# yabebalFantaye/MCEvidence

Hardware: AMD Instinct MI355X
Metric: knn_queries_per_sec (higher is better)
Workload: dtype f16 filter + f64 refine (exact f64 results)

## Files before the change

### mcevidence_amd/csrc/capi_common.hpp

```cpp
#pragma once
namespace {

thread_local char g_err[512] = "";
thread_local char g_last_kernel[256] = "";
thread_local int g_prof_on = 0;
thread_local std::vector<std::pair<hipEvent_t, hipEvent_t>> g_ev_pool;
thread_local size_t g_ev_used = 0;
thread_local size_t g_ev_calls = 0;
thread_local bool g_in_tail = false;
thread_local int g_split_depth = 0;
thread_local double g_last_prune_geom[3] = {0, 0, 0};
thread_local double g_last_flops_main = 0.0, g_last_flops_all = 0.0;
thread_local std::vector<std::pair<hipEvent_t, hipEvent_t>> g_evs_pool;
thread_local size_t g_evs_used = 0;

int fail(int code, const char* fmt, ...)
{
    va_list ap;
    va_start(ap, fmt);
    vsnprintf(g_err, sizeof(g_err), fmt, ap);
    va_end(ap);
    return code;
}

#define MCE_HIP(call)                                                                              \
    do {                                                                                           \
        hipError_t e_ = (call);                                                                    \
        if (e_ != hipSuccess)                                                                      \
            return fail(MCE_ERR_HIP, "%s failed: %s (%s:%d)", #call, hipGetErrorString(e_), __FILE__, __LINE__); \
    } while (0)

std::atomic<int> g_mode{0};
std::atomic<int> g_prune_mode{0};
struct Tuning {
    bool sym_kernel_f16 = false, tail_split = true, prune_prof = false, wide = true;
    int spin_limit = 1 << 21, sym_bucket = 0, sym_panel = 0, sym_seed_rows = 0, sym_seed_share = 2, sym_seed_mode = -1;
    int f16_seed_rows = -1, f16_seed_share = -1, f16_seed_tg = -1, rsplit = 0, panel_debug = 0, sym_chains = 0;
    size_t feed_wave_bytes = 0;
};
Tuning read_tuning()
{
    Tuning t;
    auto num = [](const char* name, int dflt) { const char* e = getenv(name); return e ? atoi(e) : dflt; };
    const char* e = getenv("MCE_SYM_KERNEL");
    t.sym_kernel_f16 = e && strcmp(e, "f16") == 0;
    t.spin_limit = num("MCE_SYM_SPIN_LIMIT", 1 << 21);
    t.sym_bucket = num("MCE_SYM_BUCKET", 0);
    t.sym_panel = num("MCE_SYM_PANEL", 0);
    t.sym_chains = num("MCE_SYM_CHAINS", 0);
    t.sym_seed_rows = num("MCE_SYM_SEED_ROWS", 0);
    t.sym_seed_share = num("MCE_SYM_SEED_SHARE", 2);
    t.sym_seed_mode = num("MCE_SYM_SEED_MODE", -1);
    t.f16_seed_rows = num("MCE_F16_SEED_ROWS", -1);
    t.f16_seed_share = num("MCE_F16_SEED_SHARE", -1);
    t.f16_seed_tg = num("MCE_F16_SEED_TG", -1);
    t.rsplit = num("MCE_RSPLIT", 0);
    t.tail_split = num("MCE_TAIL_SPLIT", 1) != 0;
    t.wide = num("MCE_WIDE", 1) != 0;
    t.panel_debug = num("MCE_PANEL_DEBUG", 0);
    t.prune_prof = getenv("MCE_PRUNE_PROF") != nullptr;
    if ((e = getenv("MCE_FEED_WAVE_BYTES"))) t.feed_wave_bytes = (size_t)std::strtoull(e, nullptr, 10);
    return t;
}
std::atomic<int> g_sym_mode{-1};
int sym_mode()
{
    int m = g_sym_mode.load();
    if (m < 0) {
        const char* e = getenv("MCE_SYM");
        m = e ? atoi(e) : 0;
        if (m < 0 || m > 2) m = 0;
        g_sym_mode.store(m);
    }
    return m;
}
const char* env_prune_heavy() { return getenv("MCE_PRUNE_HEAVY"); }
const char* env_prune_lists() { return getenv("MCE_PRUNE_LISTS"); }
const char* env_prune_times() { return getenv("MCE_PRUNE_TIMES"); }
bool env_long_on() { static const bool v = [] { const char* e = getenv("MCE_LONG"); return !(e && e[0] == '0'); }(); return v; }
bool env_deep_on() { static const bool v = [] { const char* e = getenv("MCE_DEEP"); return !(e && e[0] == '0'); }(); return v; }
int env_feed_eig() { static const int v = [] { const char* e = getenv("MCE_FEED_EIG"); return e && !strcmp(e, "hip") ? 2 : 1; }(); return v; }
bool env_feed_upload_async() { static const bool v = [] { const char* e = getenv("MCE_FEED_UPLOAD"); return e && !strcmp(e, "async"); }(); return v; }
int env_pairs_once_split() { static const int v = [] { const char* e = getenv("MCE_PAIRS_ONCE_SPLIT"); const int n = e ? atoi(e) : 0; return (n >= 1 && n <= 8) ? n : 0; }(); return v; }
int env_pairs_once_panel() { static const int v = [] { const char* e = getenv("MCE_PAIRS_ONCE_PANEL"); const int n = e ? atoi(e) : 0; return n >= 1 ? n : 0; }(); return v; }
struct CallOptions { int search = -1, prune = -1, sym = -1, same_set = -1, verify = -1, eig = 0; };
thread_local CallOptions t_opt;
thread_local std::vector<CallOptions> t_opt_stack;
int eff_search_mode() { return t_opt.search >= 0 ? t_opt.search : g_mode.load(); }
int eff_prune_mode() { return t_opt.prune >= 0 ? t_opt.prune : g_prune_mode.load(); }
int eff_sym_mode() { return t_opt.sym >= 0 ? t_opt.sym : sym_mode(); }
constexpr int kVerifyDefaultRows = 256;
constexpr int64_t kVerifyAlwaysFrom = 65536;
constexpr int kVerifySmallEvery = 8;
int default_verify_rows()
{
    static const int v = [] {
        const char* e = getenv("MCE_VERIFY");
        if (!e || !*e) return kVerifyDefaultRows;
        const long n = strtol(e, nullptr, 10);
        return (int)std::max<long>(0, std::min<long>(n, 1 << 20));
    }();
    return v;
}
bool verify_env_set() { static const bool s = [] { const char* e = getenv("MCE_VERIFY"); return e && *e; }(); return s; }
std::atomic<int> g_last_verify_rows{0};
thread_local unsigned t_small_search_count = 0;
int eff_verify(bool filter_path, int64_t nq)
{
    if (t_opt.verify >= 0) return t_opt.verify;
    if (!filter_path) return 0;
    if (nq < kVerifyAlwaysFrom && !verify_env_set() && (t_small_search_count++ % kVerifySmallEvery) != 0) return 0;
    return default_verify_rows();
}
constexpr int kSymAutoMinBlocks[5] = {0, 768, 257, 193, 193};
constexpr int kSymMaxChains = 8;
constexpr int kSymSeedMode[5] = {0, 0, 1, 1, 1};
constexpr int kSymPartitionMaxParts = 4;
thread_local int g_same_set_hint = -1;
thread_local size_t t_plan_cap = 0;
struct PlanCap {
    size_t prev;
    explicit PlanCap(size_t cap) : prev(t_plan_cap) { t_plan_cap = cap; }
    ~PlanCap() { t_plan_cap = prev; }
};
thread_local bool t_no_heavy = false;
struct NoHeavy {
    bool prev;
    NoHeavy() : prev(t_no_heavy) { t_no_heavy = true; }
    ~NoHeavy() { t_no_heavy = prev; }
};
struct SameSetHint {
    int prev;
    explicit SameSetHint(bool same) : prev(g_same_set_hint) { g_same_set_hint = same ? 1 : 0; }
    ~SameSetHint() { g_same_set_hint = prev; }
};
constexpr int kSymPanelChunks[5] = {0, 96, 256, 256, 256};
int sym_bucket_per_row(int K)
{
    const int b = read_tuning().sym_bucket;
    return b > 0 ? b : 6 * K + 24;
}
constexpr int64_t kPruneAutoMinQueries = 32768;
constexpr int64_t kPruneAutoMinRows[16] = {0, 100000, 100000, 100000, 100000, 125000, 150000, 250000, 500000, 0, 0, 0, 0, 0, 0, 0};

constexpr size_t kPoolMaxBytes = (size_t)64 << 20;
constexpr int kPoolSlots = 16;
struct PoolSlot { void* p = nullptr; size_t cap = 0; int dev = -1; bool busy = false; };
struct Pool {
    PoolSlot slot[kPoolSlots];
    PoolSlot& operator[](int i) { return slot[i]; }
    void release_idle()
    {
        for (int i = 0; i < kPoolSlots; ++i)
            if (slot[i].p && !slot[i].busy) {
                int cur = 0;
                (void)hipGetDevice(&cur);
                if (slot[i].dev != cur) (void)hipSetDevice(slot[i].dev);
                (void)hipFree(slot[i].p);
                if (slot[i].dev != cur) (void)hipSetDevice(cur);
                slot[i] = PoolSlot();
            }
    }
    ~Pool() { release_idle(); }
};
thread_local Pool g_pool;

struct PinnedArena {
    void* p = nullptr;
    size_t cap = 0;
    void release()
    {
        if (p) (void)hipHostFree(p);
        p = nullptr;
        cap = 0;
    }
    hipError_t reserve(size_t n)
    {
        if (n <= cap) return hipSuccess;
        release();
        const size_t c = std::max<size_t>(n + n / 2, (size_t)64 << 10);
        hipError_t e = hipHostMalloc(&p, c, hipHostMallocPortable);
        if (e != hipSuccess) { p = nullptr; return e; }
        cap = c;
        return hipSuccess;
    }
    ~PinnedArena() { release(); }
};
thread_local PinnedArena g_pinned;

thread_local const double* g_last_params = nullptr;

struct DevBuf {
    void* p = nullptr;
    int slot = -1;
    ~DevBuf()
    {
        if (p && g_last_params >= static_cast<const double*>(p) &&
            reinterpret_cast<const char*>(g_last_params) < static_cast<const char*>(p) + bytes)
            g_last_params = nullptr;
        if (slot >= 0) g_pool[slot].busy = false;
        else if (p) (void)hipFree(p);
    }
    size_t bytes = 0;
    hipError_t alloc(size_t n)
    {
        if (n == 0) n = 1;
        bytes = n;
        if (n <= kPoolMaxBytes) {
            int dev = 0;
            (void)hipGetDevice(&dev);
            int pick = -1;
            for (int i = 0; i < kPoolSlots; ++i)
                if (!g_pool[i].busy && g_pool[i].p && g_pool[i].dev == dev && g_pool[i].cap >= n &&
                    (pick < 0 || g_pool[i].cap < g_pool[pick].cap)) pick = i;
            if (pick < 0)
                for (int i = 0; i < kPoolSlots; ++i)
                    if (!g_pool[i].busy) {
                        if (g_pool[i].p) { (void)hipFree(g_pool[i].p); g_pool[i].p = nullptr; g_pool[i].cap = 0; }
                        const size_t cap = n + n / 4;
                        hipError_t e = hipMalloc(&g_pool[i].p, cap);
                        if (e != hipSuccess) { g_pool[i].p = nullptr; return e; }
                        g_pool[i].cap = cap;
                        g_pool[i].dev = dev;
                        pick = i;
                        break;
                    }
            if (pick >= 0) {
                g_pool[pick].busy = true;
                slot = pick;
                p = g_pool[pick].p;
                return hipSuccess;
            }
        }
        return hipMalloc(&p, n);
    }
    template <class T> T* as() { return static_cast<T*>(p); }
};

}
```

### mcevidence_amd/csrc/capi_plan.hpp

```cpp
#pragma once
namespace {

using mce::kMaxDevices;
constexpr int kAssumedCUs = 256;

size_t align_up(size_t x, size_t a) { return (x + a - 1) / a * a; }

constexpr bool kPruneHeavyDefault = false;
constexpr int kPruneHeavyMinBlocks = 64, kPruneHeavyCount = 700, kPruneHeavyMaxShare = 16, kPruneHeavyMinCount = 32, kPruneHeavyMaxRounds = 60;
constexpr double kPruneHeavyFullRounds = 10.0;
constexpr int kPruneHeavySplit = 4, kPruneHeavyMaxSplit = 8;
constexpr int kPruneWaveQueries = mce::kHQT * 32;
constexpr int kWideMinBlocks = 480;
bool prune_heavy_enabled()
{
    if (t_no_heavy) return false;
    const char* e = env_prune_heavy();
    return kPruneHeavyDefault || (e && *e && strcmp(e, "0") != 0);
}
static_assert(mce::kPruneWavesPerBlock == mce::kHWaves, "prune.hip orders kHWaves waves per query block");

constexpr int kRefineMargin = 2;
struct Plan {
    const mce::KnnVariant* v = nullptr;
    const mce::KnnF16Variant* vh = nullptr;
    const mce::KnnDeepVariant* vd = nullptr;
    bool filter() const { return vh != nullptr || vd != nullptr; }
    const mce::KnnLongVariant* vl = nullptr;
    size_t off_xf = 0, off_xn = 0;
    bool generic = false;
    int KST = 0;
    size_t off_yh = 0, off_xh = 0, off_qinfo = 0, off_params = 0;
    int KS = 0, KCAP = 0, QT = 0, CT = 0;
    int64_t nchunk = 0;
    int64_t nrow_pad = 0;
    int nqblk = 0;
    int64_t nq_pad = 0;
    int rsplit = 1;
    int L = 4;
    size_t off_yf = 0, off_pd = 0, off_pi = 0, off_center = 0, off_msum = 0, total = 0;
    double cost = 0.0;
    int ksel = 0;
    bool twopass = false;
    bool wide_ok = false;
    bool prune = false;
    bool kd_ready = false;
    int part = 0, nparts = 1;
    int sym_qb_lo = 0, sym_qb_hi = 0;
    bool apo = false;
    int apo_phase = 0;
    int apo_nsplit = 1;
    int apo_panel = 0;
    int64_t pl_nr = 0;
    mce::PruneLayout pl;
    size_t off_prune = 0;
    size_t off_heavy = 0;
    int heavy_max = 0;
    bool sym = false;
    bool sym_active = false;
    mce::SymLayout sl;
    size_t off_sym = 0;
    int sym_nsplit = 1;
    int sym_panel = 0;
};

const mce::KnnVariant* variant_for(int KS, int kcap_idx)
{
    switch (kcap_idx) {
        case 0: return &mce::g_knn_kcap4[mce::mfma_variant_index(KS)];
        case 1: return &mce::g_knn_kcap8[mce::mfma_variant_index(KS)];
        case 2: return &mce::g_knn_kcap12[mce::mfma_variant_index(KS)];
        case 3: return &mce::g_knn_kcap16[mce::mfma_variant_index(KS)];
        case 4: return &mce::g_knn_kcap24[mce::mfma_variant_index(KS)];
        default: return &mce::g_knn_kcap32[mce::mfma_variant_index(KS)];
    }
}

int sweep_seed_cfg(int64_t cps, int CT, int kneed)
{
    const Tuning t = read_tuning();
    if (t.f16_seed_rows >= 0 || t.f16_seed_share >= 0 || t.f16_seed_tg >= 0)
        return mce::f16_seed_cfg(cps, CT, kneed, t.f16_seed_rows >= 0 ? t.f16_seed_rows : MCE_H_SEED_ROWS, t.f16_seed_share >= 0 ? t.f16_seed_share : MCE_H_SEED_SHARE,
                                 t.f16_seed_tg >= 0 ? t.f16_seed_tg : MCE_H_SEED_TG);
    for (int share = MCE_H_SEED_SHARE; share >= 2; share /= 2)
        for (int tg = MCE_H_SEED_TG; tg >= 2; tg /= 2)
            if (const int cfg = mce::f16_seed_cfg(cps, CT, kneed, MCE_H_SEED_ROWS, share, tg)) return cfg;
    return 0;
}

template <class V> const V* by_kcap(int ki, const V* t4, const V* t8, const V* t12, const V* t16) { return ki == 0 ? t4 : ki == 1 ? t8 : ki == 2 ? t12 : t16; }

double split_cost(const Plan& p, bool filt, int64_t nr, int32_t K, int r)
{
    const double n_r = (double)nr / r;
    const double lnf = 1.0 + std::log(std::max(1.0, n_r / K));
    const double block = filt ? 64.0 * p.QT * p.KST * (n_r / 32.0) + 300.0 * 32.0 * p.QT * K * lnf
                              : 256.0 * p.KS * (n_r / 16.0) + 1000.0 * 32.0 * K * lnf;
    const double rounds = std::ceil((double)p.nqblk * r / kAssumedCUs);
    return rounds * block;
}

int make_plan(int64_t nq, int64_t nr, int32_t d, int32_t K, int32_t self_mode, Plan& p)
{
    if (nq < 0 || nr < 1 || d < 1 || K < 1) return fail(MCE_ERR_INVALID, "invalid sizes nq=%lld nr=%lld d=%d K=%d", (long long)nq, (long long)nr, d, K);
    if (self_mode < 0 || self_mode > 2) return fail(MCE_ERR_INVALID, "invalid self_mode %d", self_mode);
    if (d > mce::kGenMaxDim) return fail(MCE_ERR_DIM_RANGE, "d=%d exceeds the supported maximum %d", d, mce::kGenMaxDim);
    if (K > mce::kGenMaxK) return fail(MCE_ERR_K_RANGE, "K=%d exceeds the supported maximum %d", K, mce::kGenMaxK);
    const int64_t usable = (self_mode == MCE_SELF_EXCLUDE) ? nr - 1 : nr;
    if (K > usable)
        return fail(MCE_ERR_K_RANGE, "Expected n_neighbors <= n_samples_fit, but n_neighbors = %d, n_samples_fit = %lld", K, (long long)usable);
    if (nr >= (int64_t)1 << 31) return fail(MCE_ERR_INVALID, "nr=%lld exceeds 2^31-1 reference rows", (long long)nr);

    const bool wide_f64 = d > MCE_MAX_DIM && d <= mce::kWideMaxDim && K <= MCE_MAX_K;
    if (env_long_on() && d >= mce::kLongMinDim && d <= mce::kLongMaxDim && K <= MCE_MAX_K) {
        p.ksel = std::min<int>(K + kRefineMargin, MCE_MAX_K);
        p.vl = &mce::g_knn_long[p.ksel <= 8 ? 0 : (p.ksel <= 16 ? 1 : 2)];
        p.v = nullptr;
        p.vh = nullptr;
        p.KCAP = p.vl->kcap;
        p.CT = p.vl->ct;
        p.QT = mce::kLongQT;
        p.KS = mce::long_ksp(d);
        p.nqblk = (int)std::max<int64_t>(1, (nq + mce::kLongQPB - 1) / mce::kLongQPB);
        p.nq_pad = (int64_t)p.nqblk * mce::kLongQPB;
        const int64_t rows_per_chunk = (int64_t)p.CT * 16;
        p.nchunk = (nr + rows_per_chunk - 1) / rows_per_chunk;
        p.nrow_pad = p.nchunk * rows_per_chunk;
        int best_r = 1;
        double best_c = 1e300;
        const int rmax = (int)std::min<int64_t>(mce::kMaxLists, p.nchunk);
        for (int r = 1; r <= rmax; ++r) {
            const double c = std::ceil((double)p.nqblk * r / kAssumedCUs) * (std::ceil((double)p.nchunk / r) + 16.0);
            if (c < best_c * 0.98) { best_c = c; best_r = r; }
        }
        p.rsplit = best_r;
        p.L = p.rsplit;
        p.cost = best_c;
        p.pl_nr = nr;
        size_t off = 0;
        p.off_pd = off;
        off = align_up(off + (size_t)p.L * p.KCAP * (size_t)p.nq_pad * sizeof(double), 256);
        p.off_pi = off;
        off = align_up(off + (size_t)p.L * p.KCAP * (size_t)p.nq_pad * sizeof(int), 256);
        p.off_center = off;
        off = align_up(off + (size_t)(d + 4) * sizeof(double), 256);
        p.off_msum = off;
        off = align_up(off + (size_t)mce::kLongMeanBlocks * (size_t)d * sizeof(double), 256);
        p.off_yf = off;
        off = align_up(off + (size_t)p.nrow_pad * (size_t)p.KS * 4 * sizeof(double), 256);
        p.off_xf = off;
        off = align_up(off + (size_t)p.nq_pad * (size_t)p.KS * 4 * sizeof(double), 256);
        p.off_xn = off;
        off = align_up(off + (size_t)p.nq_pad * sizeof(double), 256);
        p.total = off + 256;
        return MCE_OK;
    }
    if ((d > MCE_MAX_DIM && !wide_f64) || K > MCE_MAX_K) {
        p.generic = true;
        p.v = nullptr;
        p.vh = nullptr;
        p.KCAP = K;
        p.rsplit = 1;
        p.L = 1;
        p.nqblk = (int)std::max<int64_t>(1, (nq + mce::kGenThreads - 1) / mce::kGenThreads);
        p.nq_pad = (int64_t)p.nqblk * mce::kGenThreads;
        size_t off = 0;
        p.off_pd = off;
        off = align_up(off + (size_t)K * (size_t)p.nq_pad * sizeof(double), 256);
        p.off_pi = off;
        off = align_up(off + (size_t)K * (size_t)p.nq_pad * sizeof(int), 256);
        p.off_center = off;
        off = align_up(off + (size_t)nq * K * sizeof(double), 256);
        p.off_msum = off;
        p.total = off + 256;
        return MCE_OK;
    }
    p.KS = mce::mfma_ks_for(d);
    int ki = 0;
    while (ki < mce::kNumKcap - 1 && mce::kKcapList[ki] < K) ++ki;
    p.KCAP = mce::kKcapList[ki];
    const bool f16 = !wide_f64 && (eff_search_mode() != 1) && mce::f16_supported(d, K);
    const bool deep = wide_f64 && (eff_search_mode() != 1) && mce::deep_supported(d, K) && env_deep_on();
    const bool filt = f16 || deep;
    p.vd = nullptr;
    int qpb, rows_per_tile;
    if (filt) {
        if (K > 16) {
            p.twopass = true;
            ki = 3;
            p.KCAP = 16;
        }
        if (deep) {
            p.KST = mce::deep_ksteps(d);
            p.vd = &by_kcap(ki, mce::g_knn_deep_kcap4, mce::g_knn_deep_kcap8, mce::g_knn_deep_kcap12, mce::g_knn_deep_kcap16)[p.KST == 5 ? 0 : (p.KST == 6 ? 1 : 2)];
            p.vh = nullptr;
            p.QT = mce::kHQT;
            p.CT = p.vd->ct;
        } else {
            p.KST = mce::f16_ksteps(d);
            p.vh = &by_kcap(ki, mce::g_knn_f16_kcap4, mce::g_knn_f16_kcap8, mce::g_knn_f16_kcap12, mce::g_knn_f16_kcap16)[p.KST - 1];
            p.QT = p.vh->qt;
            p.CT = p.vh->ct;
        }
        p.v = nullptr;
        qpb = mce::f16_qpb(p.KCAP);
        rows_per_tile = 32;
    } else {
        p.ksel = std::min<int>(K + kRefineMargin, MCE_MAX_K);
        p.pl_nr = nr;
        ki = 0;
        while (ki < mce::kNumKcap - 1 && mce::kKcapList[ki] < p.ksel) ++ki;
        p.KCAP = mce::kKcapList[ki];
        p.v = variant_for(p.KS, ki);
        p.vh = nullptr;
        p.QT = p.v->qt;
        p.CT = p.v->ct;
        qpb = mce::queries_per_block(p.QT);
        rows_per_tile = 16;
    }
    p.nqblk = (int)std::max<int64_t>(1, (nq + qpb - 1) / qpb);
    p.wide_ok = f16 && !p.twopass && p.KST == 1 && p.vh->launch_wide && p.nqblk >= kWideMinBlocks && nr <= ((int64_t)1 << 25) && read_tuning().wide;
    if (p.wide_ok && (p.nqblk & 1)) p.nqblk += 1;
    p.nq_pad = (int64_t)p.nqblk * qpb;
    const int64_t rows_per_chunk = (int64_t)p.CT * rows_per_tile;
    p.nchunk = (nr + rows_per_chunk - 1) / rows_per_chunk;
    p.nrow_pad = p.nchunk * rows_per_chunk;

    if (f16 && !p.twopass && p.KST == 1 && d <= mce::kPruneMaxDim && p.vh->launch_prune && nq > 0 &&
        p.nrow_pad <= ((int64_t)1 << mce::kHRelBits) && (int64_t)p.nqblk * p.nchunk <= mce::kPruneMaxPairs) {
        const int pm = eff_prune_mode();
        p.prune = pm == 2 || (pm == 0 && kPruneAutoMinRows[d] > 0 && nr >= kPruneAutoMinRows[d] && nq >= kPruneAutoMinQueries &&
                                           nq >= nr / 8);
    }
    if (p.prune) {
        p.CT = mce::kHPruneChunkTiles;
        p.nchunk = (nr + p.CT * 32 - 1) / (p.CT * 32);
        p.nrow_pad = p.nchunk * p.CT * 32;
        if (p.nrow_pad > ((int64_t)1 << mce::kHRelBits)) p.prune = false;
        if (!p.prune) {
            p.CT = p.vh->ct;
            p.nchunk = (nr + rows_per_chunk - 1) / rows_per_chunk;
            p.nrow_pad = p.nchunk * rows_per_chunk;
        }
    }
    int best_r = 1;
    double best_c = 1e300;
    const int rmax = (int)std::min<int64_t>(p.twopass ? mce::kMaxLists / 2 : mce::kMaxLists, p.nchunk);
    const int rmin = f16 ? (int)((nr + ((int64_t)1 << mce::kHRelBits) - 1) >> mce::kHRelBits) : 1;
    if (deep && p.nrow_pad > ((int64_t)1 << mce::kHRelBits))
        return fail(MCE_ERR_INVALID, "reference set too large for the fp16-filter path at d = %d (nr=%lld): use search mode 1", d, (long long)nr);
    if (rmin > rmax) return fail(MCE_ERR_INVALID, "reference set too large for the fp16-filter path (nr=%lld)", (long long)nr);
    for (int r = std::max(1, rmin); r <= rmax; ++r) {
        const double c = split_cost(p, filt, nr, K, r);
        if (c < best_c * 0.98) { best_c = c; best_r = r; }
    }
    if (f16 && !p.twopass && p.nqblk <= kAssumedCUs) {
        const int kneed = K + 1;
        for (int r = std::min(rmax, kAssumedCUs / p.nqblk); r >= std::max(1, rmin); --r)
            if (sweep_seed_cfg(p.nchunk / r, p.CT, kneed)) { best_r = r; break; }
    }
    if (deep && p.nqblk <= kAssumedCUs) {
        for (int r = std::min(rmax, kAssumedCUs / p.nqblk); r >= 1; --r)
            if ((p.nchunk / r) * p.CT >= 4 * (K + 1)) { best_r = r; break; }
    }
    if (const int r = read_tuning().rsplit) {
        if (r >= std::max(1, rmin) && r <= rmax) best_r = r;
    }
    if (p.prune) best_r = 1;
    p.rsplit = best_r;
    p.cost = split_cost(p, filt, nr, K, best_r);
    auto layout = [&]() {
    p.L = p.twopass ? 2 * p.rsplit : p.rsplit;

    size_t off = 0;
    p.off_yf = off;
    if (filt) {
        p.off_yh = off;
        off = align_up(off + (size_t)p.nrow_pad * (size_t)(16 * p.KST) * 2, 256);
        p.off_xh = off;
        off = align_up(off + (size_t)p.nq_pad * (size_t)(16 * p.KST) * 2, 256);
        p.off_qinfo = off;
        off = align_up(off + (size_t)p.nq_pad * 2 * sizeof(double), 256);
        p.off_params = off;
        off = align_up(off + (size_t)mce::HP_COUNT * sizeof(double), 256);
    } else {
        off = align_up(off + (size_t)p.nrow_pad * (size_t)(4 * p.KS) * sizeof(double), 256);
    }
    if (f16 && (!p.twopass || p.vh->launch_panel_lower) && !p.prune && nq == nr && p.vh->launch_sym && p.nqblk >= 2 && p.nrow_pad <= ((int64_t)1 << mce::kHSymRowBits)) {
        const int sm = eff_sym_mode();
        p.sym = sm == 2 || (sm == 0 && p.nqblk >= kSymAutoMinBlocks[p.KST] * ((p.KST == 1 && p.KCAP == 16) ? 2 : 1));
        if (g_same_set_hint == 0 || (g_same_set_hint < 0 && t_opt.same_set == 0)) p.sym = false;
    }
    p.sym_nsplit = 1;
    p.sym_panel = 0;
    if (p.sym && !p.twopass) {
        const Tuning tun = read_tuning();
        int S = 1;
        if (tun.sym_chains >= 1) S = std::min(tun.sym_chains, kSymMaxChains);
        p.sym_nsplit = S;
        if (S > 1) p.sym_panel = (int)std::max<int64_t>(8, std::min<int64_t>(kSymPanelChunks[p.KST], p.nchunk / (2 * S)));
    }
    const int l_alloc = std::max(p.L, p.sym_nsplit);
    p.off_pd = off;
    off = align_up(off + (size_t)l_alloc * p.KCAP * (size_t)p.nq_pad * sizeof(double), 256);
    p.off_pi = off;
    off = align_up(off + (size_t)l_alloc * p.KCAP * (size_t)p.nq_pad * sizeof(int), 256);
    p.off_center = off;
    off = align_up(off + (size_t)3 * mce::kMaxDimPad * sizeof(double), 256);
    p.off_msum = off;
    off = align_up(off + (size_t)mce::kMeanBlocks * mce::kStatStride * sizeof(double), 256);
    if (p.prune) {
        mce::prune_layout(nq, p.nq_pad, p.nqblk, nr, p.nrow_pad, p.nchunk, d, p.pl);
        p.pl_nr = nr;
        p.off_prune = off;
        off = align_up(off + p.pl.total, 256);
        if (nq == nr && p.nqblk >= kPruneHeavyMinBlocks && prune_heavy_enabled()) {
            p.heavy_max = std::max(p.nqblk * mce::kHWaves / kPruneHeavyMaxShare, kPruneHeavyMinCount);
            p.off_heavy = off;
            off = align_up(off + (size_t)p.heavy_max * kPruneWaveQueries * (kPruneHeavyMaxSplit - 1) * p.KCAP * (sizeof(double) + sizeof(int)), 256);
        }
    }
    if (p.sym) {
        mce::sym_layout(nr, p.nq_pad, p.nqblk, d, p.KCAP, mce::f16_qpb(p.KCAP), sym_bucket_per_row(std::min<int>(K, p.KCAP)), p.sl);
        p.off_sym = off;
        off = align_up(off + p.sl.total, 256);
    }
    p.total = off;
    };
    layout();
    while (t_plan_cap && p.total > t_plan_cap && p.rsplit > std::max(1, rmin)) {
        p.rsplit -= 1;
        layout();
    }
    return MCE_OK;
}

size_t dotp_ws_bytes(int64_t nq, int32_t kmax)
{
    const int64_t nb = (nq + mce::kRedThreads - 1) / mce::kRedThreads;
    return align_up((size_t)std::max<int64_t>(nb, 1) * (size_t)kmax * sizeof(double), 256);
}

int plan_for_workspace(int64_t nq, int64_t nr, int32_t d, int32_t K, int32_t self_mode, size_t ws_bytes, size_t extra, bool same_set_fallback,
                       Plan& p, std::optional<NoHeavy>& nh)
{
    int rc = make_plan(nq, nr, d, K, self_mode, p);
    if (rc != MCE_OK) return rc;
    if (same_set_fallback && ws_bytes < p.total + extra && p.sym) {
        g_same_set_hint = 0;
        rc = make_plan(nq, nr, d, K, self_mode, p);
        if (rc != MCE_OK) return rc;
    }
    if (ws_bytes < p.total + extra && p.heavy_max > 0) {
        nh.emplace();
        rc = make_plan(nq, nr, d, K, self_mode, p);
        if (rc != MCE_OK) return rc;
    }
    if (ws_bytes < p.total + extra) return fail(MCE_ERR_WORKSPACE, "workspace too small: %zu < %zu", ws_bytes, p.total + extra);
    return MCE_OK;
}

}
```

### mcevidence_amd/csrc/capi_search.hpp

```cpp
#pragma once
namespace {

double ln_unit_ball(int d) { return 0.5 * d * std::log(M_PI) - std::lgamma(1.0 + 0.5 * d); }

hipError_t launch_sym_merge(int KCAP, double* pd, int* pi, int64_t nq_pad, const mce::SymParams& sym, int qb_lo, int qb_hi, hipStream_t st, int stride = 1)
{
    const int nb = qb_hi > qb_lo ? (qb_hi - qb_lo + stride - 1) / stride : 0;
    if (nb <= 0) return hipSuccess;
    const dim3 g((unsigned)nb), b(mce::kSymMergeThreads);
    static_assert(mce::kSymMergeThreads == mce::f16_qpb(4), "one merge block per query block");
    switch (KCAP) {
        case 4: hipLaunchKernelGGL(mce::sym_merge_kernel<4>, g, b, 0, st, pd, pi, nq_pad, sym.bucket_cnt, sym.bucket_flag, sym.bucket, sym.cap, qb_lo, stride); break;
        case 8: hipLaunchKernelGGL(mce::sym_merge_kernel<8>, g, b, 0, st, pd, pi, nq_pad, sym.bucket_cnt, sym.bucket_flag, sym.bucket, sym.cap, qb_lo, stride); break;
        case 12: hipLaunchKernelGGL(mce::sym_merge_kernel<12>, g, b, 0, st, pd, pi, nq_pad, sym.bucket_cnt, sym.bucket_flag, sym.bucket, sym.cap, qb_lo, stride); break;
        default: hipLaunchKernelGGL(mce::sym_merge_kernel<16>, g, b, 0, st, pd, pi, nq_pad, sym.bucket_cnt, sym.bucket_flag, sym.bucket, sym.cap, qb_lo, stride); break;
    }
    return hipGetLastError();
}

struct KernelBracket {
    bool on = false; hipStream_t st = nullptr;
    hipError_t begin() const
    {
        if (!on) return hipSuccess;
        if (g_ev_used == g_ev_pool.size()) {
            hipEvent_t e0, e1;
            if (const hipError_t e = hipEventCreate(&e0)) return e;
            if (const hipError_t e = hipEventCreate(&e1)) return e;
            g_ev_pool.emplace_back(e0, e1);
        }
        return hipEventRecord(g_ev_pool[g_ev_used].first, st);
    }
    hipError_t end() const
    {
        if (!on) return hipSuccess;
        if (const hipError_t e = hipEventRecord(g_ev_pool[g_ev_used].second, st)) return e;
        ++g_ev_used;
        if (!g_in_tail) ++g_ev_calls;
        return hipSuccess;
    }
};
struct SearchBracket {
    hipStream_t st; bool on;
    SearchBracket(hipStream_t s, bool o) : st(s), on(o)
    {
        if (!on) return;
        if (g_evs_used == g_evs_pool.size()) {
            hipEvent_t e0, e1;
            if (hipEventCreate(&e0) != hipSuccess || hipEventCreate(&e1) != hipSuccess) { on = false; return; }
            g_evs_pool.emplace_back(e0, e1);
        }
        (void)hipEventRecord(g_evs_pool[g_evs_used].first, st);
    }
    ~SearchBracket() { if (on) { (void)hipEventRecord(g_evs_pool[g_evs_used].second, st); ++g_evs_used; } }
};

size_t list_set(const Plan& p, int set) { return (size_t)set * p.KCAP * (size_t)p.nq_pad; }

mce::KnnF16Args f16_args(const Plan& p, char* ws, const double* X, int64_t nq, const double* Y, int64_t nr, int32_t d, int32_t K, int self_exclude,
                         int64_t self_offset)
{
    mce::KnnF16Args a;
    a.Yh = ws + p.off_yh; a.nchunk_total = p.nchunk; a.rsplit = p.rsplit; a.Xh = ws + p.off_xh;
    a.qinfo = reinterpret_cast<const double*>(ws + p.off_qinfo); a.params = reinterpret_cast<const double*>(ws + p.off_params);
    a.X = X; a.Y = Y; a.nq = nq; a.nr = nr; a.D = d; a.nq_pad = p.nq_pad; a.nqblk = p.nqblk;
    a.self_exclude = self_exclude; a.self_offset = self_offset; a.ksel = K;
    a.part_d = reinterpret_cast<double*>(ws + p.off_pd); a.part_i = reinterpret_cast<int*>(ws + p.off_pi);
    return a;
}
mce::KnnF16Args sym_args(const Plan& p, char* ws, int64_t n, int32_t d, int32_t K, int self_exclude)
{
    char* const sw = ws + p.off_sym;
    const double* rows = reinterpret_cast<const double*>(sw + p.sl.Ys);
    mce::KnnF16Args a = f16_args(p, ws, rows, n, rows, n, d, K, self_exclude, 0);
    a.rsplit = 1;
    a.rperm = reinterpret_cast<const int*>(sw + p.sl.perm);
    a.sym.thr = reinterpret_cast<unsigned long long*>(sw + p.sl.thr);
    a.sym.rrow = reinterpret_cast<unsigned*>(sw + p.sl.rrow);
    a.sym.rtile = reinterpret_cast<float*>(sw + p.sl.rtile);
    a.sym.slots = reinterpret_cast<unsigned long long*>(sw + p.sl.slots);
    a.sym.bucket_cnt = reinterpret_cast<int*>(sw + p.sl.bucket_cnt);
    a.sym.bucket_flag = reinterpret_cast<int*>(sw + p.sl.bucket_flag);
    a.sym.bucket = reinterpret_cast<mce::SymEntry*>(sw + p.sl.bucket);
    a.sym.cap = p.sl.cap;
    a.sym.done = reinterpret_cast<int*>(sw + p.sl.done);
    const Tuning tun = read_tuning();
    a.sym.panel = tun.sym_panel > 0 ? tun.sym_panel : kSymPanelChunks[p.KST];
    return a;
}

struct F16Search {
    const double* sX = nullptr;
    const double* sY = nullptr;
    mce::PruneOut po;
    bool use_sym = false;
};

struct Search {
    Plan& p;
    const double* dX; int64_t nq; const double* dY; int64_t nr; int32_t d, K;
    int32_t self_mode; int64_t self_offset; char* ws; hipStream_t st;
    int phase;
    double* pd; int* pi;
    double* center; double* msum;
    int self_exclude;
    KernelBracket kb;
    int generic(), long_rows(), deep(), fp64();
    int f16_prepare(F16Search& f), pruned(const F16Search& f), symmetric(), f16_sweep(const F16Search& f);
};

int Search::generic()
{
    const size_t lds = mce::generic_lds_bytes();
    hipLaunchKernelGGL(mce::knn_generic_kernel, dim3((unsigned)p.nqblk), dim3(mce::kGenThreads), 0, st, dX, nq, dY, nr, (int)d,
                       (int)K, p.nq_pad, self_exclude, self_offset, pd, pi);
    MCE_HIP(hipGetLastError());
    snprintf(g_last_kernel, sizeof(g_last_kernel), "knn_generic_kernel grid=%d block=%d lds=%zu", p.nqblk, mce::kGenThreads, lds);
    return MCE_OK;
}

int Search::long_rows()
{
    const int threads = 256;
    double* yf = reinterpret_cast<double*>(ws + p.off_yf);
    double* xf = reinterpret_cast<double*>(ws + p.off_xf);
    double* xn = reinterpret_cast<double*>(ws + p.off_xn);
    hipLaunchKernelGGL(mce::pack_refs_kernel, dim3((unsigned)((p.nrow_pad + threads - 1) / threads)), dim3(threads), 0, st, dY, nr, (int)d, p.KS, p.nrow_pad, center, yf);
    MCE_HIP(hipGetLastError());
    const int64_t qe = p.nq_pad * (int64_t)p.KS;
    hipLaunchKernelGGL(mce::long_pack_queries_kernel, dim3((unsigned)((qe + 255) / 256)), dim3(256), 0, st, dX, nq, (int)d, p.KS, p.nq_pad, center, xf);
    MCE_HIP(hipGetLastError());
    hipLaunchKernelGGL(mce::long_query_norms_kernel, dim3((unsigned)((p.nq_pad + 255) / 256)), dim3(256), 0, st, dX, nq, (int)d, p.nq_pad, center, xn);
    MCE_HIP(hipGetLastError());
    mce::LongArgs a;
    a.Yf = yf; a.Xf = xf; a.xn = xn;
    a.nchunk_total = p.nchunk; a.rsplit = p.rsplit; a.KSP = p.KS; a.KSB = mce::long_ksb(d);
    a.nq = nq; a.nq_pad = p.nq_pad; a.nqblk = p.nqblk;
    a.self_exclude = self_exclude; a.self_offset = self_offset; a.ksel = p.ksel > K ? p.ksel : K;
    a.part_d = pd; a.part_i = pi;
    MCE_HIP(kb.begin());
    MCE_HIP(p.vl->launch(a, st));
    MCE_HIP(kb.end());
    snprintf(g_last_kernel, sizeof(g_last_kernel), "%s grid=%d block=%d lds=%zu qt=%d ct=%d rsplit=%d ksp=%d", p.vl->name, p.nqblk * p.rsplit, mce::kThreads,
             p.vl->lds_bytes, p.QT, p.CT, p.rsplit, p.KS);
    g_last_flops_main = g_last_flops_all = (double)p.nq_pad * (double)p.nrow_pad * 2.0 * 4.0 * p.KS;
    return MCE_OK;
}

int Search::deep()
{
    _Float16* yh = reinterpret_cast<_Float16*>(ws + p.off_yh);
    _Float16* xh = reinterpret_cast<_Float16*>(ws + p.off_xh);
    double* qinfo = reinterpret_cast<double*>(ws + p.off_qinfo);
    double* params = reinterpret_cast<double*>(ws + p.off_params);
    MCE_HIP(mce::zero_async(params, mce::HP_COUNT * sizeof(double), st));
    const bool separate_queries = !(dX >= dY && dX + (size_t)nq * d <= dY + (size_t)nr * d);
    hipLaunchKernelGGL(mce::f16_radius_rows_kernel, dim3((unsigned)std::min<int64_t>((nr + 255) / 256, 2048)), dim3(256), 0, st, dY, nr, (int)d, center, params);
    MCE_HIP(hipGetLastError());
    if (separate_queries && nq > 0) {
        hipLaunchKernelGGL(mce::f16_radius_rows_kernel, dim3((unsigned)std::min<int64_t>((nq + 255) / 256, 2048)), dim3(256), 0, st, dX, nq, (int)d, center, params);
        MCE_HIP(hipGetLastError());
    }
    hipLaunchKernelGGL(mce::f16_scale_from_radius_kernel, dim3(1), dim3(1), 0, st, params);
    MCE_HIP(hipGetLastError());
    const int64_t rows_per_block = 4 * (64 / (2 * p.KST));
    const int64_t pack_blocks = std::min<int64_t>((p.nrow_pad + rows_per_block - 1) / rows_per_block, 2048);
    hipLaunchKernelGGL(mce::f16_pack_refs_kernel, dim3((unsigned)pack_blocks), dim3(256), 0, st, dY, nr, (int)d, p.KST, p.nrow_pad, center, params, yh);
    MCE_HIP(hipGetLastError());
    hipLaunchKernelGGL(mce::f16_pack_queries_kernel, dim3((unsigned)((p.nq_pad + rows_per_block - 1) / rows_per_block)), dim3(256), 0, st,
                       dX, nq, p.nq_pad, (int)d, p.KST, center, params, xh, qinfo);
    MCE_HIP(hipGetLastError());
    mce::DeepArgs a;
    a.Yh = yh; a.Xh = xh; a.qinfo = qinfo; a.params = params; a.X = dX; a.Y = dY; a.part_d = pd; a.part_i = pi;
    a.nq = nq; a.nr = nr; a.nq_pad = p.nq_pad; a.self_offset = self_offset; a.nchunk_total = p.nchunk;
    a.D = d; a.ksel = K; a.self_exclude = self_exclude; a.nqblk = p.nqblk; a.rsplit = p.rsplit;
    const Tuning tun = read_tuning();
    a.debug = tun.panel_debug;
    const int64_t tiles_split = (p.nchunk / p.rsplit) * p.CT;
    const int64_t want = (tun.f16_seed_rows >= 0 ? tun.f16_seed_rows : MCE_H_SEED_ROWS) / 32;
    auto tg_for = [&](int G) {
        int64_t tg = std::min<int64_t>(want, tiles_split / 4) / G;
        if (tg < 1) tg = std::min<int64_t>(want, tiles_split / 2) / G;
        return (int)std::max<int64_t>(tg, 0);
    };
    a.seed_tg = tg_for(K + a.self_exclude);
    MCE_HIP(kb.begin());
    double seed_rows = (double)a.seed_tg * (K + a.self_exclude) * 32.0 * p.rsplit;
    if (p.twopass) {
        const int tg2 = a.seed_tg;
        a.ksel = 16;
        a.seed_groups = 16 + a.self_exclude;
        a.seed_tg = tg_for(a.seed_groups);
        const int tg1 = a.seed_tg;
        MCE_HIP(p.vd->launch(a, st));
        a.lo_d = pd; a.lo_i = pi;
        a.part_d = pd + list_set(p, p.rsplit); a.part_i = pi + list_set(p, p.rsplit);
        a.ksel = K - 16;
        a.seed_groups = K + a.self_exclude;
        a.seed_tg = tg2;
        MCE_HIP(p.vd->launch_lower(a, st));
        seed_rows = ((double)tg1 * (16 + a.self_exclude) + (double)tg2 * (K + a.self_exclude)) * 32.0 * p.rsplit;
    } else {
        MCE_HIP(p.vd->launch(a, st));
    }
    MCE_HIP(kb.end());
    g_last_flops_main = g_last_flops_all = (double)p.nq_pad * ((p.twopass ? 2.0 : 1.0) * (double)p.nrow_pad + seed_rows) * 2.0 * 16.0 * p.KST;
    snprintf(g_last_kernel, sizeof(g_last_kernel), "%s grid=%d block=%d lds=%zu qt=%d ct=%d rsplit=%d%s seed=%dx%d", p.vd->name, p.nqblk * p.rsplit, mce::kHThreads,
             p.vd->lds_bytes, p.QT, p.CT, p.rsplit, p.twopass ? " two passes" : "", K + a.self_exclude, a.seed_tg);
    return MCE_OK;
}

int Search::f16_prepare(F16Search& f)
{
    _Float16* yh = reinterpret_cast<_Float16*>(ws + p.off_yh);
    _Float16* xh = reinterpret_cast<_Float16*>(ws + p.off_xh);
    double* qinfo = reinterpret_cast<double*>(ws + p.off_qinfo);
    double* params = reinterpret_cast<double*>(ws + p.off_params);
    double* box_y = center + mce::kMaxDimPad;
    double* box_x = center + 2 * mce::kMaxDimPad;
    if (phase != 2) MCE_HIP(mce::zero_async(params, mce::HP_COUNT * sizeof(double), st));
    bool separate_queries = !(dX >= dY && dX + (size_t)nq * d <= dY + (size_t)nr * d);
    f.sX = dX; f.sY = dY;
    f.use_sym = p.sym && dX == dY && nq == nr && self_offset == 0 && g_split_depth == 0;
    if (f.use_sym) {
        if (phase != 2) MCE_HIP(mce::sym_prepare(dY, nr, (int)d, center, p.nq_pad, ws + p.off_sym, p.sl, st));
        f.sX = f.sY = reinterpret_cast<const double*>(ws + p.off_sym + p.sl.Ys);
        separate_queries = false;
    }
    if (p.prune) {
        const bool same_set = (dX == dY && nq == nr);
        MCE_HIP(mce::prune_prepare(dX, nq, dY, nr, (int)d, same_set, mce::f16_qpb(p.KCAP), p.CT * 32, p.nq_pad, p.nqblk, p.nrow_pad,
                                   p.nchunk, ws + p.off_prune, p.pl, st, f.po, p.kd_ready && same_set));
        f.sX = f.po.Xs; f.sY = f.po.Ys;
        separate_queries = separate_queries && !same_set;
    }
    if (separate_queries) {
        hipLaunchKernelGGL(mce::col_stats_partial_kernel, dim3(mce::kMeanBlocks), dim3(mce::kMeanThreads), 0, st, dX, nq, (int)d, msum);
        MCE_HIP(hipGetLastError());
        hipLaunchKernelGGL(mce::f16_box_about_kernel, dim3(1), dim3(64), 0, st, msum, (int)d, center, box_x);
        MCE_HIP(hipGetLastError());
    }
    if (phase == 2) return MCE_OK;
    hipLaunchKernelGGL(mce::f16_scale_kernel, dim3(1), dim3(64), 0, st, box_y, separate_queries ? box_x : (const double*)nullptr, params);
    MCE_HIP(hipGetLastError());
    const int64_t rows_per_block = 4 * (64 / (2 * p.KST));
    const int64_t pack_blocks = std::min<int64_t>((p.nrow_pad + rows_per_block - 1) / rows_per_block, 2048);
    const bool one_pass = f.sX == f.sY && nq == nr && p.nq_pad <= p.nrow_pad;
    hipLaunchKernelGGL(mce::f16_pack_refs_kernel, dim3((unsigned)pack_blocks), dim3(256), 0, st,
                       f.sY, nr, (int)d, p.KST, p.nrow_pad, center, params, yh, one_pass ? xh : (_Float16*)nullptr, one_pass ? qinfo : (double*)nullptr,
                       one_pass ? p.nq_pad : (int64_t)0);
    MCE_HIP(hipGetLastError());
    if (!one_pass) {
        hipLaunchKernelGGL(mce::f16_pack_queries_kernel, dim3((unsigned)((p.nq_pad + rows_per_block - 1) / rows_per_block)), dim3(256), 0, st,
                           f.sX, nq, p.nq_pad, (int)d, p.KST, center, params, xh, qinfo);
        MCE_HIP(hipGetLastError());
    }
    return MCE_OK;
}

int Search::pruned(const F16Search& f)
{
    const mce::PruneOut& po = f.po;
    mce::KnnF16Args a = f16_args(p, ws, f.sX, nq, f.sY, nr, d, K, self_exclude, self_offset);
    a.clist = po.clist; a.cdist = po.cdist; a.list_len = (int)p.nchunk; a.rperm = po.rperm; a.qperm = po.qperm;
    a.tbox_r = po.tbox_r; a.tbox_q = po.tbox_q; a.cbox_r = po.cbox_r; a.border = po.border;
    const int nw_total = p.nqblk * mce::kHWaves;
    if (p.nparts > 1) { a.qblk0 = p.part; a.qblk_stride = p.nparts; a.nqblk_run = (nw_total - p.part + p.nparts - 1) / p.nparts; }
    const int nblk_run = a.nqblk_run ? a.nqblk_run : nw_total;
    int hv_n = 0, hv_S = 1;
    if (p.heavy_max > 0 && dX == dY && nq == nr) {
        const double rounds = (double)nblk_run / 2048.0;
        const char* hv_env = env_prune_heavy();
        if ((kPruneHeavyDefault || (hv_env && !strcmp(hv_env, "auto"))) && rounds < kPruneHeavyMaxRounds) {
            const double fr = std::min(1.0, kPruneHeavyFullRounds / std::max(rounds, 1.0));
            hv_n = std::min(std::max((int)(kPruneHeavyCount * fr), kPruneHeavyMinCount), std::min(p.heavy_max, nblk_run));
            hv_S = kPruneHeavySplit;
        }
        if (const char* e = hv_env) {
            int n_ = hv_n, s_ = kPruneHeavySplit;
            if (sscanf(e, "%d,%d", &n_, &s_) >= 1) { hv_n = std::min(std::max(n_, 0), std::min(p.heavy_max, nblk_run)); hv_S = std::min(std::max(s_, 1), kPruneHeavyMaxSplit); }
        }
        if (hv_n == 0 || hv_S == 1) { hv_n = 0; hv_S = 1; }
    }
    double* hv_d = reinterpret_cast<double*>(ws + p.off_heavy);
    int* hv_i = reinterpret_cast<int*>(hv_d + (size_t)p.heavy_max * kPruneWaveQueries * (kPruneHeavyMaxSplit - 1) * p.KCAP);
    a.seed_cfg = hv_n | (hv_S << 24);
    a.lo_d = hv_n ? hv_d : nullptr; a.lo_i = hv_n ? hv_i : nullptr;
    const char* times_file = env_prune_times();
    const size_t n_wg = (size_t)(nblk_run + hv_n * (hv_S - 1));
    DevBuf wg_times;
    if (times_file && *times_file) { MCE_HIP(wg_times.alloc(n_wg * sizeof(float))); a.wg_us = wg_times.as<float>(); }
    MCE_HIP(kb.begin());
    const char* force_lists = env_prune_lists();
    mce::knn_f16_launch_fn short_fn = nullptr;
    int short_lc = 0;
    if (p.vh->launch_prune_short && K <= p.vh->prune_short_lc) { short_fn = p.vh->launch_prune_short; short_lc = p.vh->prune_short_lc; }
    else if (p.vh->launch_prune_short2 && K <= p.vh->prune_short_lc2) { short_fn = p.vh->launch_prune_short2; short_lc = p.vh->prune_short_lc2; }
    const bool short_lists = short_fn && !(force_lists && !strcmp(force_lists, "long"));
    MCE_HIP(short_lists ? short_fn(a, st) : p.vh->launch_prune(a, st));
    MCE_HIP(kb.end());
    if (a.wg_us) {
        std::vector<float> us(n_wg);
        MCE_HIP(hipStreamSynchronize(st));
        MCE_HIP(hipMemcpy(us.data(), a.wg_us, n_wg * sizeof(float), hipMemcpyDeviceToHost));
        if (FILE* fh = fopen(times_file, "wb")) {
            const int hdr[4] = {(int)n_wg, hv_n, hv_S, 1};
            fwrite(hdr, sizeof(int), 4, fh);
            fwrite(us.data(), sizeof(float), n_wg, fh);
            fclose(fh);
        }
    }
    if (hv_n) {
        const unsigned fb = (unsigned)(((int64_t)hv_n * kPruneWaveQueries + mce::kRedThreads - 1) / mce::kRedThreads);
        hipLaunchKernelGGL(mce::prune_heavy_fold_kernel, dim3(fb), dim3(mce::kRedThreads), 0, st, pd, pi, p.nq_pad, p.KCAP, hv_d, hv_i, hv_n, hv_S,
                           kPruneWaveQueries, po.border, a.qblk0, a.qblk_stride);
        MCE_HIP(hipGetLastError());
    }
    g_last_params = a.params;
    g_last_flops_main = g_last_flops_all = -1.0;
    g_last_prune_geom[0] = p.nqblk; g_last_prune_geom[1] = (double)p.nchunk; g_last_prune_geom[2] = p.CT;
    snprintf(g_last_kernel, sizeof(g_last_kernel), "%s pruned grid=%d block=64 lds=%zu qt=%d ct=%d chunks=%lld heavy=%dx%d lists=%d", p.vh->name,
             nblk_run + hv_n * (hv_S - 1), mce::f16_prune_lds_bytes(p.KST, d, short_lists ? short_lc : p.KCAP), p.QT, p.CT, (long long)p.nchunk, hv_n,
             hv_S, short_lists ? short_lc : p.KCAP);
    return MCE_OK;
}

int sym_units_and_flops(const Plan& p, const mce::PanelGeom& g, bool panel_kernel, int64_t nr, int panel)
{
    int units = mce::sym_unit_count(p.nqblk, mce::kHWaves * mce::kHQT, panel * p.CT, (int)((nr + 31) / 32) + (int)(((nr + 31) / 32) & 1));
    double tiles = 0.0;
    if (panel_kernel) {
        units = mce::panel_unit_count(g);
        for (int u = 0; g_prof_on && u < units; ++u) {
            int pp, aa, lo, hi;
            mce::panel_unit_decode(u, g, pp, aa);
            mce::panel_unit_tiles(pp, aa, g, lo, hi);
            tiles += hi - lo;
        }
    } else {
        const double tpb = mce::kHWaves * mce::kHQT, T = (double)((nr + 31) / 32);
        for (int b = 0; b < p.nqblk; ++b) tiles += std::min(tpb * (b + 1), T);
    }
    g_last_flops_main = tiles * 16.0 * 1024.0 * 32.0 * p.KST;
    return units;
}

int Search::symmetric()
{
    char* const sw = ws + p.off_sym;
    mce::KnnF16Args a = sym_args(p, ws, nr, d, K, self_exclude);
    const Tuning tun = read_tuning();
    const int seed_rows = tun.sym_seed_rows > 0 ? tun.sym_seed_rows : (p.KST == 1 ? 65536 : 32768) * (p.apo && p.nparts >= 4 ? 2 : 1);
    const int seed_share = tun.sym_seed_share;
    auto sym_seed_for = [&](int kk) {
        int cfg = mce::f16_seed_cfg(p.nchunk, p.CT, kk + a.self_exclude, seed_rows, seed_share, MCE_H_SEED_TG);
        for (int tg = MCE_H_SEED_TG / 2; cfg == 0 && tg >= 1; tg /= 2)
            cfg = mce::f16_seed_cfg(p.nchunk, p.CT, kk + a.self_exclude, seed_rows, seed_share, tg);
        if (cfg) cfg |= ((tun.sym_seed_mode >= 0 ? tun.sym_seed_mode : kSymSeedMode[p.KST]) & 3) << 28;
        return cfg;
    };
    const int qb_lo = p.nparts > 1 && !p.apo ? (int)((int64_t)p.nqblk * p.part / p.nparts) : 0;
    const int qb_hi = p.nparts > 1 && !p.apo ? (int)((int64_t)p.nqblk * (p.part + 1) / p.nparts) : p.nqblk;
    p.sym_qb_lo = qb_lo; p.sym_qb_hi = qb_hi;
    const bool panel_kernel = !tun.sym_kernel_f16 || p.nparts > 1 || p.twopass;
    mce::PanelGeom geom;
    geom.qb_lo = qb_lo; geom.qb_hi = qb_hi; geom.tpb = mce::kHWaves * mce::kHQT; geom.ct = p.CT; geom.tpp = a.sym.panel * p.CT; geom.sym_on = 1;
    geom.ntiles = (int)((nr + 31) / 32) + (int)(((nr + 31) / 32) & 1);
    const bool apo = p.apo && p.nparts > 1 && !p.twopass && panel_kernel;
    const bool chains1 = !apo && p.nparts == 1 && panel_kernel && !p.twopass && p.sym_nsplit > 1;
    if (apo) { geom.blk_first = p.part; geom.blk_stride = p.nparts; }
    if (apo || chains1) {
        const int pn = apo ? p.apo_panel : p.sym_panel;
        if (pn > 0 && (apo || tun.sym_panel <= 0)) { a.sym.panel = pn; geom.tpp = a.sym.panel * p.CT; }
        geom.nsplit = std::max(1, apo ? p.apo_nsplit : p.sym_nsplit);
        if (geom.nsplit > 1) {
            a.sym.done = reinterpret_cast<int*>(sw + p.sl.keys_b);
            MCE_HIP(mce::zero_async(a.sym.done, (size_t)p.nqblk * geom.nsplit * sizeof(int), st));
            if (!apo) {
                hipLaunchKernelGGL(mce::sym_chain_init_kernel, dim3((unsigned)p.nqblk), dim3(512), 0, st, pd, pi, p.nq_pad, p.KCAP, geom.nsplit, 0, 1);
                MCE_HIP(hipGetLastError());
            }
        }
    }
    const bool unit_table = apo || geom.nsplit > 1;
    const int npass = p.twopass ? 2 : 1;
    int seed_used = 0;
    for (int pass = 0; pass < npass; ++pass) {
        const bool lower = pass == 1;
        const int Kp = !p.twopass ? K : (lower ? K - 16 : 16);
        double* const pdp = pd + (lower ? list_set(p, 1) : 0);
        int* const pip = pi + (lower ? list_set(p, 1) : 0);
        if (lower) {
            MCE_HIP(mce::zero_async(a.sym.bucket_cnt, (size_t)3 * p.nqblk * sizeof(int), st));
            a.sym.slot_stride = p.KCAP;
        }
        a.ksel = lower ? K : Kp;
        a.seed_cfg = sym_seed_for(a.ksel);
        a.part_d = pdp; a.part_i = pip;
        a.qblk0 = qb_lo;
        a.nqblk_run = qb_hi - qb_lo;
        if (apo) {
            a.qblk0 = p.part; a.qblk_stride = p.nparts; a.nqblk_run = mce::apo_rank_count(p.nqblk, p.part, p.nparts);
        }
        if (a.nqblk_run > 0 && phase != 2) MCE_HIP((lower ? p.vh->launch_sym_pre32 : p.vh->launch_sym_pre)(a, st));
        a.qblk0 = 0; a.qblk_stride = 1; a.nqblk_run = 0;
        if (phase == 1) return MCE_OK;
        if (pass == 0) seed_used = a.seed_cfg;
        a.seed_cfg = 0;
        a.ksel = Kp;
        a.lo_d = lower ? pd : nullptr; a.lo_i = lower ? pi : nullptr;
        if (pass == 0) MCE_HIP(kb.begin());
        if (panel_kernel) {
            mce::PanelArgs pa;
            pa.Yh = static_cast<const _Float16*>(a.Yh); pa.Xh = static_cast<const _Float16*>(a.Xh); pa.qinfo = a.qinfo; pa.params = a.params;
            pa.X = a.X; pa.Y = a.Y; pa.rperm = a.rperm;
            pa.part_d = pdp; pa.part_i = pip; pa.nq = nq; pa.nr = nr; pa.nq_pad = p.nq_pad; pa.self_offset = 0;
            pa.D = d; pa.ksel = Kp; pa.self_exclude = a.self_exclude; pa.spin_limit = tun.spin_limit;
            pa.sym = a.sym; pa.debug = tun.panel_debug; pa.geom = geom; pa.lo_d = a.lo_d; pa.lo_i = a.lo_i;
            if (unit_table) {
                const int nun = mce::panel_unit_count(geom);
                if ((size_t)nun * sizeof(mce::PanelUnit) > (size_t)p.nq_pad * sizeof(int)) return fail(MCE_ERR_INVALID, "symmetric sweep: %d units do not fit the table", nun);
                mce::PanelUnit* tab = reinterpret_cast<mce::PanelUnit*>(sw + p.sl.vals_a);
                if (nun > 0) {
                    hipLaunchKernelGGL(mce::panel_unit_table_kernel, dim3((unsigned)((nun + 255) / 256)), dim3(256), 0, st, geom, nun, tab);
                    MCE_HIP(hipGetLastError());
                }
                pa.units = tab;
            }
            MCE_HIP((lower ? p.vh->launch_panel_lower : p.vh->launch_panel)(pa, st));
        } else {
            MCE_HIP(p.vh->launch_sym(a, st));
        }
        if (pass == 0) MCE_HIP(kb.end());
        if (apo) break;
        MCE_HIP((lower ? p.vh->launch_sym_repair_lower : p.vh->launch_sym_repair)(a, st));
        if (geom.nsplit > 1) {
            hipLaunchKernelGGL(mce::sym_chain_clear_kernel, dim3((unsigned)p.nqblk), dim3(512), 0, st, a.sym.bucket_flag, pdp, pip, p.nq_pad, p.KCAP, geom.nsplit, 0, 1);
            MCE_HIP(hipGetLastError());
        }
        MCE_HIP(launch_sym_merge(p.KCAP, pdp, pip, p.nq_pad, a.sym, qb_lo, qb_hi, st));
    }
    p.sym_active = true;
    p.L = geom.nsplit > 1 ? geom.nsplit : npass;
    const int sym_units = sym_units_and_flops(p, geom, panel_kernel, nr, a.sym.panel);
    g_last_flops_all = g_last_flops_main + (double)(seed_used & 0xffff) * p.CT * (double)(qb_hi - qb_lo) * 16.0 * 1024.0 * 32.0 * p.KST;
    snprintf(g_last_kernel, sizeof(g_last_kernel), "%s symmetric%s%s%s grid=%d block=%d lds=%zu qt=%d ct=%d panel=%d seed=%dx%d/%d bucket=%d", p.vh->name, panel_kernel ? " panel-kernel" : "",
             p.twopass ? " two passes" : "", geom.blk_stride > 1 ? " pairs-once" : (geom.nsplit > 1 ? " chains" : ""), sym_units,
             mce::kHThreads, panel_kernel ? p.vh->lds_bytes_panel : p.vh->lds_bytes_sym, p.QT, p.CT, a.sym.panel, seed_used & 0xffff, (seed_used >> 16) & 0xfff, (seed_used >> 28) & 3, p.sl.cap);
    return MCE_OK;
}

int Search::f16_sweep(const F16Search& f)
{
    mce::KnnF16Args a = f16_args(p, ws, f.sX, nq, f.sY, nr, d, K, self_exclude, self_offset);
    auto seed_cfg = [&](int ksel) { return sweep_seed_cfg(p.nchunk / p.rsplit, p.CT, ksel + a.self_exclude); };
    MCE_HIP(kb.begin());
    if (p.twopass) {
        a.ksel = 16;
        a.seed_cfg = seed_cfg(16);
        MCE_HIP(p.vh->launch(a, st));
        a.lo_d = pd; a.lo_i = pi;
        a.part_d = pd + list_set(p, p.rsplit); a.part_i = pi + list_set(p, p.rsplit);
        a.ksel = K - 16;
        a.seed_cfg = 0;
        MCE_HIP(p.vh->launch_lower(a, st));
    } else {
        a.seed_cfg = seed_cfg(K);
        if (p.wide_ok) MCE_HIP(p.vh->launch_wide(a, st));
        else MCE_HIP(p.vh->launch(a, st));
    }
    MCE_HIP(kb.end());
    const int seed_first = p.twopass ? seed_cfg(16) : a.seed_cfg;
    g_last_flops_main = (double)p.nqblk * ((double)p.nchunk + (double)(seed_first & 0xffff) * p.rsplit) * p.CT * 16.0 * 1024.0 * 32.0 * p.KST +
                        (p.twopass ? (double)p.nqblk * (double)p.nchunk * p.CT * 16.0 * 1024.0 * 32.0 * p.KST : 0.0);
    g_last_flops_all = g_last_flops_main;
    char seed_txt[48] = "";
    if (seed_first) snprintf(seed_txt, sizeof(seed_txt), " seed=%dx%d", seed_first & 0xffff, seed_first >> 16);
    const bool wide = p.wide_ok && !p.twopass;
    snprintf(g_last_kernel, sizeof(g_last_kernel), "%s grid=%d block=%d lds=%zu qt=%d ct=%d rsplit=%d%s%s%s", p.vh->name,
             (wide ? p.nqblk / 2 : p.nqblk) * p.rsplit, mce::kHThreads, wide ? p.vh->lds_bytes_wide : p.vh->lds_bytes, wide ? 2 * p.QT : p.QT, p.CT, p.rsplit,
             p.twopass ? " two passes" : "", seed_txt, wide ? " wide" : "");
    return MCE_OK;
}

int Search::fp64()
{
    const int threads = 256;
    double* yf = reinterpret_cast<double*>(ws + p.off_yf);
    hipLaunchKernelGGL(mce::pack_refs_kernel, dim3((unsigned)((p.nrow_pad + threads - 1) / threads)), dim3(threads), 0, st, dY, nr,
                       (int)d, p.KS, p.nrow_pad, center, yf);
    MCE_HIP(hipGetLastError());
    mce::KnnArgs a;
    a.Yf = yf; a.nchunk_total = p.nchunk; a.rsplit = p.rsplit; a.X = dX; a.center = center; a.nq = nq; a.D = d;
    a.nq_pad = p.nq_pad; a.nqblk = p.nqblk; a.self_exclude = self_exclude; a.self_offset = self_offset;
    a.ksel = p.ksel > K ? p.ksel : K;
    a.part_d = pd; a.part_i = pi;
    MCE_HIP(kb.begin());
    MCE_HIP(p.v->launch(a, st));
    MCE_HIP(kb.end());
    snprintf(g_last_kernel, sizeof(g_last_kernel), "%s grid=%d block=%d lds=%zu qt=%d ct=%d rsplit=%d", p.v->name,
             p.nqblk * p.rsplit, mce::kThreads, p.v->lds_bytes, p.QT, p.CT, p.rsplit);
    g_last_flops_main = g_last_flops_all = (double)p.nq_pad * (double)p.nrow_pad * 2.0 * 4.0 * p.KS;
    return MCE_OK;
}

int run_search(Plan& p, const double* dX, int64_t nq, const double* dY, int64_t nr, int32_t d, int32_t K,
               int32_t self_mode, int64_t self_offset, char* ws, hipStream_t st)
{
    p.sym_active = false;
    const int phase = p.apo ? p.apo_phase : 0;
    double* center = reinterpret_cast<double*>(ws + p.off_center);
    double* msum = reinterpret_cast<double*>(ws + p.off_msum);
    Search s{p, dX, nq, dY, nr, d, K, self_mode, self_offset, ws, st, phase, reinterpret_cast<double*>(ws + p.off_pd), reinterpret_cast<int*>(ws + p.off_pi),
             center, msum, (self_mode == MCE_SELF_EXCLUDE) ? 1 : 0, KernelBracket{}};
    if (p.generic) return s.generic();
    if (p.vl) {
        hipLaunchKernelGGL(mce::long_col_mean_partial_kernel, dim3(mce::kLongMeanBlocks), dim3(256), 0, st, dY, nr, (int)d, mce::kLongMeanBlocks, msum);
        MCE_HIP(hipGetLastError());
        hipLaunchKernelGGL(mce::long_col_mean_final_kernel, dim3((unsigned)((d + 255) / 256)), dim3(256), 0, st, msum, nr, (int)d, mce::kLongMeanBlocks, center);
        MCE_HIP(hipGetLastError());
    } else if (d > MCE_MAX_DIM) {
        static_assert(3 * mce::kMaxDimPad >= 128 && mce::kStatStride >= 128, "wide column means");
        hipLaunchKernelGGL(mce::col_mean_wide_partial_kernel, dim3(mce::kMeanBlocks), dim3(256), 0, st, dY, nr, (int)d, msum);
        MCE_HIP(hipGetLastError());
        hipLaunchKernelGGL(mce::col_mean_wide_final_kernel, dim3(1), dim3(128), 0, st, msum, nr, (int)d, center);
        MCE_HIP(hipGetLastError());
    } else if (phase != 2) {
        hipLaunchKernelGGL(mce::col_stats_partial_kernel, dim3(mce::kMeanBlocks), dim3(mce::kMeanThreads), 0, st, dY, nr, (int)d, msum);
        MCE_HIP(hipGetLastError());
        hipLaunchKernelGGL(mce::col_stats_final_kernel, dim3(1), dim3(64), 0, st, msum, nr, (int)d, center, center + mce::kMaxDimPad);
        MCE_HIP(hipGetLastError());
    }
    const bool prof = g_prof_on && g_ev_used < 1024;
    SearchBracket search_bracket(st, prof && g_evs_used < 1024);
    g_last_flops_main = g_last_flops_all = 0.0;
    s.kb = KernelBracket{prof, st};
    if (p.vl) return s.long_rows();
    if (p.vd) return s.deep();
    if (!p.vh) return s.fp64();
    F16Search f;
    const int rc = s.f16_prepare(f);
    if (rc != MCE_OK) return rc;
    if (p.prune) return s.pruned(f);
    return f.use_sym ? s.symmetric() : s.f16_sweep(f);
}

int launch_merge(const Plan& p, bool write_dist, bool fuse, const double* dX, const double* dY, int64_t nq, int32_t d, int K,
                 int self_mode, int64_t self_offset, double* d_dist, int64_t* d_idx, int k0, int kmax,
                 const double* d_w, const double* d_fs, double* partial, char* ws, hipStream_t st)
{
    const bool same_set = (dX == dY && nq == p.pl_nr);
    const bool wave_parts = p.prune && p.nparts > 1 && !p.sym_active;
    const int qpb = wave_parts ? kPruneWaveQueries : (p.filter() ? mce::f16_qpb(p.KCAP) : 1);
    const int nunits = wave_parts ? p.nqblk * mce::kHWaves : p.nqblk;
    int64_t ncol = nq;
    int64_t col0 = 0, col1 = INT64_MAX;
    const int* border = p.prune ? reinterpret_cast<const int*>(ws + p.off_prune + p.pl.border) : nullptr;
    if (p.sym_active && p.nparts > 1 && p.apo) {
        ncol = (int64_t)((nunits - p.part + p.nparts - 1) / p.nparts) * qpb;
        border = reinterpret_cast<const int*>(ws + p.off_sym + p.sl.done);
    } else if (p.sym_active && p.nparts > 1) {
        col0 = (int64_t)p.sym_qb_lo * qpb;
        col1 = std::min<int64_t>((int64_t)p.sym_qb_hi * qpb, nq);
        ncol = std::max<int64_t>(col1 - col0, 0);
    } else if (p.nparts > 1) ncol = (int64_t)((nunits - p.part + p.nparts - 1) / p.nparts) * qpb;
    const unsigned blocks = (unsigned)std::max<int64_t>((ncol + mce::kRedThreads - 1) / mce::kRedThreads, 1);
    const double* pd = reinterpret_cast<const double*>(ws + p.off_pd);
    const int* pi = reinterpret_cast<const int*>(ws + p.off_pi);
    const bool refine = !p.filter() && !p.generic;
    const double lnc = fuse ? ln_unit_ball(d) : 0.0;
    const int* qperm = nullptr;
    if (p.prune) qperm = reinterpret_cast<const int*>(ws + p.off_prune + (same_set ? p.pl.perm_r : p.pl.perm_q));
    if (p.sym_active) qperm = reinterpret_cast<const int*>(ws + p.off_sym + p.sl.perm);
#define MCE_MERGE(W, F, R)                                                                                          \
    hipLaunchKernelGGL((mce::merge_lists_kernel<W, F, R>), dim3(blocks), dim3(mce::kRedThreads), 0, st, pd, pi, p.L,  \
                       p.KCAP, nq, p.nq_pad, dX, dY, (int)d, K, (refine && p.ksel > K) ? p.ksel : K, self_mode, self_offset, d_dist, d_idx, K, k0, kmax, \
                       d_w, d_fs, lnc, partial, qperm, p.part, p.nparts, qpb, border, nunits, col0, col1, p.pl_nr, \
                       refine ? reinterpret_cast<const double*>(ws + p.off_center) : nullptr)
    if (write_dist && !fuse) { if (refine) MCE_MERGE(true, false, true); else MCE_MERGE(true, false, false); }
    else if (write_dist && fuse) { if (refine) MCE_MERGE(true, true, true); else MCE_MERGE(true, true, false); }
    else { if (refine) MCE_MERGE(false, true, true); else MCE_MERGE(false, true, false); }
#undef MCE_MERGE
    MCE_HIP(hipGetLastError());
    return MCE_OK;
}

int finish_dotp(const double* partial, int64_t ncols, int k0, int kmax, double* d_dotp, hipStream_t st)
{
    const unsigned blocks = (unsigned)std::max<int64_t>((ncols + mce::kRedThreads - 1) / mce::kRedThreads, 1);
    hipLaunchKernelGGL(mce::dotp_final_kernel, dim3((unsigned)kmax), dim3(mce::kRedThreads), 0, st, partial, (int64_t)blocks, k0, kmax, d_dotp);
    MCE_HIP(hipGetLastError());
    return MCE_OK;
}
int zero_dotp(double* d_dotp, int kmax, hipStream_t st) { MCE_HIP(mce::zero_async(d_dotp, (size_t)kmax * sizeof(double), st)); return MCE_OK; }

}
```

### mcevidence_amd/csrc/f16_filter.hpp

```cpp
#pragma once
#include <math.h>
#include <stdint.h>
#if defined(__HIPCC__)
#include <hip/hip_runtime.h>
#endif

#include "sym_types.hpp"

namespace mce {

#if defined(__HIPCC__)
#define MCE_HDI __host__ __device__ __forceinline__
#else
#define MCE_HDI inline
#endif

enum { HP_RMAX = 0, HP_SCALE = 1, HP_EY = 2, HP_YHATMAX = 3, HP_RHO = 4, HP_STAT_CHUNKS = 5, HP_STAT_TILES = 6, HP_COUNT = 16 };

constexpr int kHWaves = 8;
constexpr int kHThreads = kHWaves * 64;
constexpr int kHRelBits = 26;
constexpr int kHSymRowBits = kHRelBits - 1;

MCE_HDI float f16_round_up(double g)
{
#if defined(__HIP_DEVICE_COMPILE__)
    return __double2float_ru(g);
#else
    float f = (float)g;
    if ((double)f < g) f = nextafterf(f, __builtin_huge_valf());
    return f;
#endif
}
struct F16GateTerms { double a, c, eps; };
MCE_HDI double f16_gate_a(double ex, double ey, int KST) { return (ex + ey) * (1.0 + 1e-9) + 2.0 * sqrt(16.0 * KST) * 0x1p-14; }
MCE_HDI F16GateTerms f16_gate_terms(double ex, double xn, double ey, double ymax, double rho, int KST, bool live = true)
{
    const double r = sqrt(xn) + ymax;
    const double a = f16_gate_a(ex, ey, KST);
    const double eps = (32.0 * KST) * 0x1p-24 * r * r * (1.0 + 0x1p-9) + rho + 1e-30;
    return {a, live ? eps - xn : -__builtin_huge_val(), eps};
}
MCE_HDI double f16_reach2(double thr, double s2, double a)
{
    const double rr = sqrt(thr * s2) * (1.0 + 1e-12) + a;
    return rr * rr * (1.0 + 1e-12);
}
MCE_HDI float f16_gate_finite(double thr, double s2, double a, double c) { return f16_round_up(f16_reach2(thr, s2, a) + c); }
MCE_HDI float f16_gate(double thr, double s2, double a, double c)
{
    if (!(c > -__builtin_huge_val())) return -__builtin_huge_valf();
    if (!(thr < __builtin_huge_val())) return __builtin_huge_valf();
    return f16_gate_finite(thr, s2, a, c);
}
MCE_HDI double f16_row_const(double ymax) { return 0x1p-22 * (ymax * ymax + 1.0); }
MCE_HDI float f16_row_round(double g, double rowc) { return f16_round_up(g * (1.0 + 0x1p-22) + rowc + 1e-30); }
MCE_HDI float f16_row_gate(double thr, double s2, double a, double rowc)
{
    if (!(thr < __builtin_huge_val())) return __builtin_huge_valf();
    return f16_row_round(f16_reach2(thr, s2, a), rowc);
}
template <class P>
MCE_HDI float f16_row_gate_of(double thr, double ex, P params, int KST)
{
    if (!(thr < __builtin_huge_val())) return __builtin_huge_valf();
    const double s2 = params[HP_SCALE] * params[HP_SCALE];
    const double g = f16_reach2(thr, s2, f16_gate_a(ex, params[HP_EY], KST));
    return f16_row_round(g, f16_row_const(params[HP_YHATMAX]));
}
MCE_HDI double f16_seed_bound(double a_up, double xn, double eps, double a, double s2)
{
    const double dd = sqrt(fmax(a_up + xn + eps, 0.0)) * (1.0 + 1e-12) + a;
    return dd * dd * (1.0 + 1e-12) / s2 * (1.0 + 1e-12);
}

template <int N, class D, class I>
MCE_HD inline void list_insert(D&& own_d, I&& own_i, double d2, int j)
{
    const double INF = __builtin_huge_val();
    bool c_hi = (d2 < own_d[N - 1]) || (d2 == own_d[N - 1] && j < own_i[N - 1] && d2 < INF);
#pragma unroll
    for (int k = N - 1; k >= 1; --k) {
        const bool c_lo = (d2 < own_d[k - 1]) || (d2 == own_d[k - 1] && j < own_i[k - 1] && d2 < INF);
        own_d[k] = c_lo ? own_d[k - 1] : (c_hi ? d2 : own_d[k]);
        own_i[k] = c_lo ? own_i[k - 1] : (c_hi ? j : own_i[k]);
        c_hi = c_lo;
    }
    own_d[0] = c_hi ? d2 : own_d[0];
    own_i[0] = c_hi ? j : own_i[0];
}

#if defined(__HIPCC__)
typedef _Float16 v8h __attribute__((ext_vector_type(8)));
typedef float v16f __attribute__((ext_vector_type(16)));

__device__ __forceinline__ float min3f(float a, float b, float c)
{
    float r;
    asm("v_min3_f32 %0, %1, %2, %3" : "=v"(r) : "v"(a), "v"(b), "v"(c));
    return r;
}
__device__ __forceinline__ void f16_min16_halves(const v16f& c, float (&l1)[5], float& m0, float& m3)
{
    l1[0] = min3f(c[0], c[1], c[2]);
    l1[1] = min3f(c[3], c[4], c[5]);
    l1[2] = min3f(c[6], c[7], c[8]);
    l1[3] = min3f(c[9], c[10], c[11]);
    l1[4] = min3f(c[12], c[13], c[14]);
    m0 = min3f(l1[0], l1[1], l1[2]);
    m3 = min3f(l1[3], l1[4], c[15]);
}
__device__ __forceinline__ float f16_min16(const v16f& c, float (&l1)[5])
{
    float m0, m3;
    f16_min16_halves(c, l1, m0, m3);
    return min3f(m0, m3, m3);
}
__device__ __forceinline__ float f16_min16(const v16f& c, float (&l1)[5], float run)
{
    float m0, m3;
    f16_min16_halves(c, l1, m0, m3);
    return min3f(run, m0, m3);
}

template <int KCAP, class PS, class PT, class PR, class PF, class RG>
__device__ __forceinline__ bool sym_slot_insert(PS slots, PT thr, PR rrow, PF rtile, int ksel, int row, double d2, RG row_gate)
{
    const auto sl = slots + (int64_t)row * KCAP;
    for (;;) {
        double vmax = -1.0, v2 = -1.0;
        int imax = 0;
#pragma unroll
        for (int k = 0; k < KCAP; ++k) {
            if (k < ksel) {
                const double v = __longlong_as_double((long long)__hip_atomic_load(sl + k, __ATOMIC_RELAXED, __HIP_MEMORY_SCOPE_AGENT));
                if (v > vmax) { v2 = vmax; vmax = v; imax = k; }
                else if (v > v2) v2 = v;
            }
        }
        if (d2 > vmax) return false;
        if (d2 == vmax) return true;
        unsigned long long expect = (unsigned long long)__double_as_longlong(vmax);
        if (__hip_atomic_compare_exchange_strong(sl + imax, &expect, (unsigned long long)__double_as_longlong(d2), __ATOMIC_RELAXED,
                                                 __ATOMIC_RELAXED, __HIP_MEMORY_SCOPE_AGENT)) {
            const double nk = fmax(v2, d2);
            if (nk < __builtin_huge_val()) {
                const unsigned long long nb = (unsigned long long)__double_as_longlong(nk);
                const unsigned long long ob = __hip_atomic_fetch_min(thr + row, nb, __ATOMIC_RELAXED, __HIP_MEMORY_SCOPE_AGENT);
                if (nb < ob) {
                    const unsigned rb = __float_as_uint(row_gate(nk, row));
                    const unsigned orb = __hip_atomic_fetch_min(rrow + row, rb, __ATOMIC_RELAXED, __HIP_MEMORY_SCOPE_AGENT);
                    if (rb < orb) {
                        const auto rt = rrow + (int64_t)(row >> 5) * 32;
                        unsigned m = 0;
                        for (int k = 0; k < 32; ++k) {
                            const unsigned v = __hip_atomic_load(rt + k, __ATOMIC_RELAXED, __HIP_MEMORY_SCOPE_AGENT);
                            m = v > m ? v : m;
                        }
                        __hip_atomic_store(rtile + (row >> 5), __uint_as_float(m), __ATOMIC_RELAXED, __HIP_MEMORY_SCOPE_AGENT);
                    }
                }
            }
            return true;
        }
    }
}

template <bool ROWFLAG>
__device__ __forceinline__ unsigned f16_event(const v16f& c, const float (&l1)[5], const unsigned lanew, const float g, const bool rowflag, const int jb0,
                                              const unsigned todo, const int qlimit, int* const wq, int& qcount)
{
    const unsigned wbase = (lanew + (unsigned)jb0) | (ROWFLAG && rowflag ? (1u << kHSymRowBits) : 0u);
    unsigned rem = 0;
#define MCE_HIT(R_, P_, S_)                                                                                               \
    if ((S_) != 0 && (todo & (1u << (R_)))) {                                                                             \
        if (qcount > qlimit) rem |= 1u << (R_);                                                                           \
        else {                                                                                                            \
            if (P_) wq[__builtin_amdgcn_mbcnt_hi((unsigned)((S_) >> 32), __builtin_amdgcn_mbcnt_lo((unsigned)(S_), (unsigned)qcount))] = \
                        (int)(wbase + (unsigned)(((R_) & 3) + 8 * ((R_) >> 2)));                                          \
            qcount += __builtin_popcountll(S_);                                                                           \
        }                                                                                                                 \
    }
#define MCE_TRIPLE(I_, U_)                                                                                                \
    if ((U_) != 0) {                                                                                                      \
        const bool p0 = c[3 * (I_) + 0] <= g, p1 = c[3 * (I_) + 1] <= g, p2 = c[3 * (I_) + 2] <= g;                     \
        const unsigned long long s0 = __ballot(p0), s1 = __ballot(p1), s2 = __ballot(p2);                                \
        MCE_HIT(3 * (I_) + 0, p0, s0)                                                                                     \
        MCE_HIT(3 * (I_) + 1, p1, s1)                                                                                     \
        MCE_HIT(3 * (I_) + 2, p2, s2)                                                                                     \
    }
    const bool q0 = l1[0] <= g, q1 = l1[1] <= g, q2 = l1[2] <= g, q3 = l1[3] <= g, q4 = l1[4] <= g, p15 = c[15] <= g;
    const unsigned long long u0 = __ballot(q0), u1 = __ballot(q1), u2 = __ballot(q2), u3 = __ballot(q3), u4 = __ballot(q4), s15 = __ballot(p15);
    MCE_TRIPLE(0, u0) MCE_TRIPLE(1, u1) MCE_TRIPLE(2, u2) MCE_TRIPLE(3, u3) MCE_TRIPLE(4, u4)
    MCE_HIT(15, p15, s15)
#undef MCE_TRIPLE
#undef MCE_HIT
    return rem;
}

template <int VPT, class P>
__device__ __forceinline__ void f16_stage_chunk(P src, char* dst, int tid, int wave)
{
#pragma unroll
    for (int i = 0; i < VPT; ++i) {
        const int e = tid + i * kHThreads;
        __builtin_amdgcn_global_load_lds(
            (const __attribute__((address_space(1))) void*)(src + (size_t)e * 16),
            (__attribute__((address_space(3))) void*)(dst + (size_t)(wave * 64 + i * kHThreads) * 16),
            16, 0, 0);
    }
}
template <int KST>
__device__ __forceinline__ void f16_load_a(const char* lp, v8h (&a)[KST])
{
#pragma unroll
    for (int ks = 0; ks < KST; ++ks) a[ks] = *reinterpret_cast<const v8h*>(lp + ks * 1024);
}

#endif

}
```

### mcevidence_amd/csrc/knn_dispatch.hpp

```cpp
#pragma once
#include <hip/hip_runtime.h>
#include <stdint.h>

#include "sym_types.hpp"

namespace mce {

constexpr int kMaxDevices = 64;

struct KnnArgs {
    const double* Yf;
    int64_t nchunk_total;
    int rsplit;
    const double* X;
    const double* center;
    int64_t nq;
    int D;
    int64_t nq_pad;
    int nqblk;
    int self_exclude;
    int64_t self_offset;
    int ksel;
    double* part_d;
    int* part_i;
};

typedef hipError_t (*knn_launch_fn)(const KnnArgs&, hipStream_t);

struct KnnVariant {
    knn_launch_fn launch;
    int ks, kcap, qt, ct;
    size_t lds_bytes;
    const char* name;
};

struct KnnF16Args {
    const void* Yh;
    int64_t nchunk_total;
    int rsplit;
    const void* Xh;
    const double* qinfo;
    const double* params;
    const double* X;
    const double* Y;
    int64_t nq, nr;
    int D;
    int64_t nq_pad;
    int nqblk;
    int self_exclude;
    int64_t self_offset;
    int ksel;
    double* part_d;
    int* part_i;
    const int* clist = nullptr;
    const float* cdist = nullptr;
    int list_len = 0;
    const int* rperm = nullptr;
    const int* qperm = nullptr;
    const float* tbox_r = nullptr;
    const float* tbox_q = nullptr;
    const float* cbox_r = nullptr;
    const double* lo_d = nullptr;
    const int* lo_i = nullptr;
    int seed_cfg = 0;
    const int* border = nullptr;
    int qblk0 = 0, qblk_stride = 1, nqblk_run = 0;
    SymParams sym;
    float* wg_us = nullptr;
};
typedef hipError_t (*knn_f16_launch_fn)(const KnnF16Args&, hipStream_t);
struct PanelArgs;
typedef hipError_t (*knn_panel_launch_fn)(const PanelArgs&, hipStream_t);
struct KnnF16Variant {
    knn_f16_launch_fn launch;
    knn_f16_launch_fn launch_prune;
    knn_f16_launch_fn launch_lower;
    knn_f16_launch_fn launch_sym_pre;
    knn_f16_launch_fn launch_sym;
    knn_f16_launch_fn launch_sym_repair;
    knn_panel_launch_fn launch_panel;
    size_t lds_bytes_panel;
    size_t lds_bytes_sym;
    int kst, kcap, qt, ct;
    size_t lds_bytes;
    const char* name;
    knn_f16_launch_fn launch_prune_short;
    int prune_short_lc;
    knn_f16_launch_fn launch_prune_short2;
    int prune_short_lc2;
    knn_f16_launch_fn launch_wide;
    size_t lds_bytes_wide;
    knn_panel_launch_fn launch_panel_lower;
    knn_f16_launch_fn launch_sym_repair_lower;
    knn_f16_launch_fn launch_sym_pre32;
};
struct DeepArgs;
typedef hipError_t (*knn_deep_launch_fn)(const DeepArgs&, hipStream_t);
struct KnnDeepVariant {
    knn_deep_launch_fn launch;
    int kst, kcap, ct;
    size_t lds_bytes;
    const char* name;
    knn_deep_launch_fn launch_lower;
};
struct LongArgs;
typedef hipError_t (*knn_long_launch_fn)(const LongArgs&, hipStream_t);
struct KnnLongVariant {
    knn_long_launch_fn launch;
    int kcap, ct;
    size_t lds_bytes;
    const char* name;
};
constexpr int kNumLongKcap = 3;
extern const KnnLongVariant g_knn_long[kNumLongKcap];
constexpr int kNumDeepKST = 3;
extern const KnnDeepVariant g_knn_deep_kcap4[kNumDeepKST];
extern const KnnDeepVariant g_knn_deep_kcap8[kNumDeepKST];
extern const KnnDeepVariant g_knn_deep_kcap12[kNumDeepKST];
extern const KnnDeepVariant g_knn_deep_kcap16[kNumDeepKST];

constexpr int kMaxKST = 4;
extern const KnnF16Variant g_knn_f16_kcap4[kMaxKST];
extern const KnnF16Variant g_knn_f16_kcap8[kMaxKST];
extern const KnnF16Variant g_knn_f16_kcap12[kMaxKST];
extern const KnnF16Variant g_knn_f16_kcap16[kMaxKST];

constexpr int kMaxKS = 20;
constexpr int kWideMaxDim = 127;
__host__ __device__ constexpr int mfma_ks_for(int d) { return d <= 63 ? (d + 1 + 3) / 4 : ((d + 1 + 15) / 16) * 4; }
__host__ __device__ constexpr int mfma_variant_index(int KS) { return KS <= 16 ? KS - 1 : 11 + KS / 4; }
constexpr int kNumKcap = 6;
constexpr int kKcapList[kNumKcap] = {4, 8, 12, 16, 24, 32};

extern const KnnVariant g_knn_kcap4[kMaxKS];
extern const KnnVariant g_knn_kcap8[kMaxKS];
extern const KnnVariant g_knn_kcap12[kMaxKS];
extern const KnnVariant g_knn_kcap16[kMaxKS];
extern const KnnVariant g_knn_kcap24[kMaxKS];
extern const KnnVariant g_knn_kcap32[kMaxKS];

}
```

### mcevidence_amd/csrc/knn_inst.hip

```cpp
#include "knn_mfma.hpp"
#include "knn_f16.hpp"
#include "knn_panel.hpp"
#include "knn_deep.hpp"
#include "knn_dispatch.hpp"

#ifndef MCE_KCAP
#error "compile with -DMCE_KCAP=n"
#endif
#ifndef MCE_INST_PART
#define MCE_INST_PART 0
#endif
#define MCE_INST_F16 (MCE_KCAP <= 16 && (MCE_INST_PART == 0 || MCE_INST_PART == 1))
#define MCE_INST_F64 (MCE_INST_PART == 0 || MCE_INST_PART == 2)
#define MCE_INST_PANEL (MCE_KCAP <= 16 && (MCE_INST_PART == 0 || MCE_INST_PART == 3))
#define MCE_INST_DEEP (MCE_KCAP <= 16 && (MCE_INST_PART == 0 || MCE_INST_PART == 4))

namespace mce {

#if MCE_INST_F64
template <int KS, int KCAP>
hipError_t launch_variant(const KnnArgs& a, hipStream_t st)
{
    constexpr size_t LDS = lds_bytes(KS, KCAP);
    static_assert(LDS <= 160 * 1024, "LDS budget");
    static bool attr_set[kMaxDevices] = {};
    auto kern = knn_mfma_kernel<KS, KCAP>;
    int dev = 0;
    (void)hipGetDevice(&dev);
    if (dev >= kMaxDevices || !attr_set[dev]) {
        hipError_t e = hipFuncSetAttribute(reinterpret_cast<const void*>(kern), hipFuncAttributeMaxDynamicSharedMemorySize, (int)LDS);
        if (e != hipSuccess) return e;
        if (dev < kMaxDevices) attr_set[dev] = true;
    }
    const dim3 grid((unsigned)(a.nqblk * a.rsplit));
    hipLaunchKernelGGL(kern, grid, dim3(kThreads), LDS, st, a.Yf, a.nchunk_total, a.rsplit, a.X, a.center, a.nq, a.D,
                       a.nq_pad, a.nqblk, a.self_exclude, a.self_offset, a.ksel, a.part_d, a.part_i);
    return hipGetLastError();
}
#endif

#if MCE_INST_F16
template <int KST, int KCAP, bool PRUNE, bool LOWER = false, int SYM = 0, int LC = KCAP, int QTT = kHQT>
hipError_t launch_f16_variant(const KnnF16Args& a, hipStream_t st)
{
    constexpr size_t LDS_MAX = PRUNE ? f16_prune_lds_bytes(KST, 16 * KST - 1, LC) : f16_lds_bytes(KST, KCAP, SYM >= 2, QTT);
    static_assert(LDS_MAX <= 160 * 1024, "LDS budget");
    const size_t LDS = PRUNE ? f16_prune_lds_bytes(KST, a.D, LC) : LDS_MAX;
    static bool attr_set[kMaxDevices] = {};
    auto kern = knn_f16_kernel<KST, KCAP, PRUNE, LOWER, SYM, LC, QTT>;
    constexpr int WB = QTT / kHQT;
    int dev = 0;
    (void)hipGetDevice(&dev);
    if (dev >= kMaxDevices || !attr_set[dev]) {
        hipError_t e = hipFuncSetAttribute(reinterpret_cast<const void*>(kern), hipFuncAttributeMaxDynamicSharedMemorySize, (int)LDS_MAX);
        if (e != hipSuccess) return e;
        if (dev < kMaxDevices) attr_set[dev] = true;
    }
    const int ntiles_even = (int)((a.nr + 31) / 32) + (int)(((a.nr + 31) / 32) & 1);
    const int hv_n = PRUNE ? (a.seed_cfg & 0xffffff) : 0, hv_S = PRUNE && ((a.seed_cfg >> 24) & 0x7f) > 1 ? ((a.seed_cfg >> 24) & 0x7f) : 1;
    const dim3 grid((unsigned)(PRUNE ? (a.nqblk_run ? a.nqblk_run : a.nqblk * kHWaves) + hv_n * (hv_S - 1)
                               : SYM == 2 ? sym_unit_count(a.nqblk, kHWaves * kHQT, a.sym.panel * f16_chunk_tiles(KST), ntiles_even)
                               : SYM == 1 ? (a.nqblk_run ? a.nqblk_run : a.nqblk) : (a.nqblk / WB) * a.rsplit));
    hipLaunchKernelGGL(kern, grid, dim3(PRUNE ? 64 : kHThreads), LDS, st, static_cast<const _Float16*>(a.Yh), a.nchunk_total, a.rsplit,
                       static_cast<const _Float16*>(a.Xh), a.qinfo, a.params, a.X, a.Y, a.nq, a.nr, a.D, a.nq_pad, a.nqblk / WB,
                       a.self_exclude, a.self_offset, a.ksel, a.part_d, a.part_i, a.clist, a.cdist, a.list_len, a.rperm, a.qperm, a.tbox_r, a.tbox_q, a.cbox_r, a.qblk0, a.qblk_stride, a.border, a.lo_d, a.lo_i, a.seed_cfg, a.sym, a.wg_us);
    return hipGetLastError();
}
#endif

#if MCE_INST_F16 || MCE_INST_PANEL
template <int KST, int KCAP, bool LOWER = false>
hipError_t launch_panel_variant(const PanelArgs& a, hipStream_t st)
#if MCE_INST_PANEL
{
    constexpr size_t LDS = panel_lds_bytes(KST);
    static_assert(LDS <= 160 * 1024, "LDS budget");
    static bool attr_set[kMaxDevices] = {};
    auto kern = knn_panel_kernel<KST, KCAP, LOWER>;
    int dev = 0;
    (void)hipGetDevice(&dev);
    if (dev >= kMaxDevices || !attr_set[dev]) {
        hipError_t e = hipFuncSetAttribute(reinterpret_cast<const void*>(kern), hipFuncAttributeMaxDynamicSharedMemorySize, (int)LDS);
        if (e != hipSuccess) return e;
        if (dev < kMaxDevices) attr_set[dev] = true;
    }
    const int units = panel_unit_count(a.geom);
    if (units <= 0) return hipSuccess;
    hipLaunchKernelGGL(kern, dim3((unsigned)units), dim3(kHThreads), LDS, st, a);
    return hipGetLastError();
}
template hipError_t launch_panel_variant<1, MCE_KCAP>(const PanelArgs&, hipStream_t);
template hipError_t launch_panel_variant<2, MCE_KCAP>(const PanelArgs&, hipStream_t);
template hipError_t launch_panel_variant<3, MCE_KCAP>(const PanelArgs&, hipStream_t);
template hipError_t launch_panel_variant<4, MCE_KCAP>(const PanelArgs&, hipStream_t);
#if MCE_KCAP == 16
template hipError_t launch_panel_variant<1, MCE_KCAP, true>(const PanelArgs&, hipStream_t);
template hipError_t launch_panel_variant<2, MCE_KCAP, true>(const PanelArgs&, hipStream_t);
template hipError_t launch_panel_variant<3, MCE_KCAP, true>(const PanelArgs&, hipStream_t);
template hipError_t launch_panel_variant<4, MCE_KCAP, true>(const PanelArgs&, hipStream_t);
#endif
#else
;
extern template hipError_t launch_panel_variant<1, MCE_KCAP>(const PanelArgs&, hipStream_t);
extern template hipError_t launch_panel_variant<2, MCE_KCAP>(const PanelArgs&, hipStream_t);
extern template hipError_t launch_panel_variant<3, MCE_KCAP>(const PanelArgs&, hipStream_t);
extern template hipError_t launch_panel_variant<4, MCE_KCAP>(const PanelArgs&, hipStream_t);
#if MCE_KCAP == 16
extern template hipError_t launch_panel_variant<1, MCE_KCAP, true>(const PanelArgs&, hipStream_t);
extern template hipError_t launch_panel_variant<2, MCE_KCAP, true>(const PanelArgs&, hipStream_t);
extern template hipError_t launch_panel_variant<3, MCE_KCAP, true>(const PanelArgs&, hipStream_t);
extern template hipError_t launch_panel_variant<4, MCE_KCAP, true>(const PanelArgs&, hipStream_t);
#endif
#endif
#endif

#if MCE_INST_DEEP
template <int KST, int KCAP, bool LOWER = false>
hipError_t launch_deep_variant(const DeepArgs& a, hipStream_t st)
{
    constexpr size_t LDS = deep_lds_bytes(KST);
    static_assert(LDS <= 160 * 1024, "LDS budget");
    static bool attr_set[kMaxDevices] = {};
    auto kern = knn_deep_kernel<KST, KCAP, LOWER>;
    int dev = 0;
    (void)hipGetDevice(&dev);
    if (dev >= kMaxDevices || !attr_set[dev]) {
        hipError_t e = hipFuncSetAttribute(reinterpret_cast<const void*>(kern), hipFuncAttributeMaxDynamicSharedMemorySize, (int)LDS);
        if (e != hipSuccess) return e;
        if (dev < kMaxDevices) attr_set[dev] = true;
    }
    hipLaunchKernelGGL(kern, dim3((unsigned)(a.nqblk * a.rsplit)), dim3(kHThreads), LDS, st, a);
    return hipGetLastError();
}
#endif

#define MCE_STR2(x) #x
#define MCE_STR(x) MCE_STR2(x)
#define MCE_VARIANT(KS)                                                                                  \
    {&launch_variant<KS, MCE_KCAP>, KS, MCE_KCAP, mfma_qt(KS), chunk_tiles(KS, MCE_KCAP), lds_bytes(KS, MCE_KCAP),  \
     "knn_mfma_kernel<KS=" #KS ",KCAP=" MCE_STR(MCE_KCAP) ">"}

#define MCE_CAT2(a, b) a##b
#define MCE_CAT(a, b) MCE_CAT2(a, b)

#if !defined(__HIP_DEVICE_COMPILE__)
#if MCE_INST_F64
extern const KnnVariant MCE_CAT(g_knn_kcap, MCE_KCAP)[kMaxKS] = {
    MCE_VARIANT(1),  MCE_VARIANT(2),  MCE_VARIANT(3),  MCE_VARIANT(4),  MCE_VARIANT(5),  MCE_VARIANT(6),
    MCE_VARIANT(7),  MCE_VARIANT(8),  MCE_VARIANT(9),  MCE_VARIANT(10), MCE_VARIANT(11), MCE_VARIANT(12),
    MCE_VARIANT(13), MCE_VARIANT(14), MCE_VARIANT(15), MCE_VARIANT(16),
    MCE_VARIANT(20), MCE_VARIANT(24), MCE_VARIANT(28), MCE_VARIANT(32),
};
#endif
#if MCE_INST_F16
#if MCE_KCAP == 16
#define MCE_F16_LOWER(KST) (&launch_f16_variant<KST, MCE_KCAP, false, true>)
#define MCE_F16_SYM_LOWER(KST) &launch_panel_variant<KST, MCE_KCAP, true>, &launch_f16_variant<KST, MCE_KCAP, false, true, 3>, &launch_f16_variant<KST, 32, false, false, 1>
#else
#define MCE_F16_LOWER(KST) nullptr
#define MCE_F16_SYM_LOWER(KST) nullptr, nullptr, nullptr
#endif
#if MCE_KCAP == 12
#define MCE_F16_SHORT(KST) ((KST) == 1 ? &launch_f16_variant<1, MCE_KCAP, true, false, 0, 9> : (knn_f16_launch_fn) nullptr), ((KST) == 1 ? 9 : 0), \
                           ((KST) == 1 ? &launch_f16_variant<1, MCE_KCAP, true, false, 0, 10> : (knn_f16_launch_fn) nullptr), ((KST) == 1 ? 10 : 0)
#else
#define MCE_F16_SHORT(KST) nullptr, 0, nullptr, 0
#endif
#if MCE_KCAP == 4
#define MCE_F16_WIDE(KST) ((KST) == 1 ? &launch_f16_variant<1, MCE_KCAP, false, false, 0, MCE_KCAP, 4> : (knn_f16_launch_fn) nullptr), ((KST) == 1 ? f16_lds_bytes(1, MCE_KCAP, false, 4) : 0)
#else
#define MCE_F16_WIDE(KST) nullptr, 0
#endif
#define MCE_F16_VARIANT(KST, PRUNE_FN)                                                                   \
    {&launch_f16_variant<KST, MCE_KCAP, false>, PRUNE_FN, MCE_F16_LOWER(KST), &launch_f16_variant<KST, MCE_KCAP, false, false, 1>, \
     &launch_f16_variant<KST, MCE_KCAP, false, false, 2>, &launch_f16_variant<KST, MCE_KCAP, false, false, 3>, &launch_panel_variant<KST, MCE_KCAP>, panel_lds_bytes(KST), \
     f16_lds_bytes(KST, MCE_KCAP, true), KST, MCE_KCAP, f16_qt(MCE_KCAP), f16_chunk_tiles(KST), \
     f16_lds_bytes(KST, MCE_KCAP), "knn_f16_kernel<KST=" #KST ",KCAP=" MCE_STR(MCE_KCAP) ">", MCE_F16_SHORT(KST), MCE_F16_WIDE(KST), MCE_F16_SYM_LOWER(KST)}
extern const KnnF16Variant MCE_CAT(g_knn_f16_kcap, MCE_KCAP)[kMaxKST] = {
    MCE_F16_VARIANT(1, (&launch_f16_variant<1, MCE_KCAP, true>)), MCE_F16_VARIANT(2, nullptr), MCE_F16_VARIANT(3, nullptr),
    MCE_F16_VARIANT(4, nullptr),
};
#endif
#if MCE_INST_DEEP
#if MCE_KCAP == 16
#define MCE_DEEP_LOWER(KST) (&launch_deep_variant<KST, MCE_KCAP, true>)
#else
#define MCE_DEEP_LOWER(KST) nullptr
#endif
#define MCE_DEEP_VARIANT(KST) {&launch_deep_variant<KST, MCE_KCAP>, KST, MCE_KCAP, deep_chunk_tiles(KST), deep_lds_bytes(KST), "knn_deep_kernel<KST=" #KST ",KCAP=" MCE_STR(MCE_KCAP) ">", MCE_DEEP_LOWER(KST)}
extern const KnnDeepVariant MCE_CAT(g_knn_deep_kcap, MCE_KCAP)[kNumDeepKST] = {MCE_DEEP_VARIANT(5), MCE_DEEP_VARIANT(6), MCE_DEEP_VARIANT(8)};
#endif
#else
#if MCE_INST_DEEP
template __global__ void knn_deep_kernel<5, MCE_KCAP>(DeepArgs);
template __global__ void knn_deep_kernel<6, MCE_KCAP>(DeepArgs);
template __global__ void knn_deep_kernel<8, MCE_KCAP>(DeepArgs);
#if MCE_KCAP == 16
template __global__ void knn_deep_kernel<5, MCE_KCAP, true>(DeepArgs);
template __global__ void knn_deep_kernel<6, MCE_KCAP, true>(DeepArgs);
template __global__ void knn_deep_kernel<8, MCE_KCAP, true>(DeepArgs);
#endif
#endif
#if MCE_INST_F16
#define MCE_F16_INST(KST, PR, LW, SY) template __global__ void knn_f16_kernel<KST, MCE_KCAP, PR, LW, SY>(const _Float16*, int64_t, int, const _Float16*, const double*, const double*, const double*, const double*, int64_t, int64_t, int, int64_t, int, int, int64_t, int, double*, int*, const int*, const float*, int, const int*, const int*, const float*, const float*, const float*, int, int, const int*, const double*, const int*, int, SymParams, float*);
MCE_F16_INST(1, false, false, 0) MCE_F16_INST(2, false, false, 0) MCE_F16_INST(3, false, false, 0) MCE_F16_INST(4, false, false, 0) MCE_F16_INST(1, true, false, 0)
MCE_F16_INST(1, false, false, 1) MCE_F16_INST(2, false, false, 1) MCE_F16_INST(3, false, false, 1) MCE_F16_INST(4, false, false, 1)
MCE_F16_INST(1, false, false, 2) MCE_F16_INST(2, false, false, 2) MCE_F16_INST(3, false, false, 2) MCE_F16_INST(4, false, false, 2)
MCE_F16_INST(1, false, false, 3) MCE_F16_INST(2, false, false, 3) MCE_F16_INST(3, false, false, 3) MCE_F16_INST(4, false, false, 3)
#if MCE_KCAP == 12
template __global__ void knn_f16_kernel<1, MCE_KCAP, true, false, 0, 9>(const _Float16*, int64_t, int, const _Float16*, const double*, const double*, const double*, const double*, int64_t, int64_t, int, int64_t, int, int, int64_t, int, double*, int*, const int*, const float*, int, const int*, const int*, const float*, const float*, const float*, int, int, const int*, const double*, const int*, int, SymParams, float*);
template __global__ void knn_f16_kernel<1, MCE_KCAP, true, false, 0, 10>(const _Float16*, int64_t, int, const _Float16*, const double*, const double*, const double*, const double*, int64_t, int64_t, int, int64_t, int, int, int64_t, int, double*, int*, const int*, const float*, int, const int*, const int*, const float*, const float*, const float*, int, int, const int*, const double*, const int*, int, SymParams, float*);
#endif
#if MCE_KCAP == 16
MCE_F16_INST(1, false, true, 0) MCE_F16_INST(2, false, true, 0) MCE_F16_INST(3, false, true, 0) MCE_F16_INST(4, false, true, 0)
MCE_F16_INST(1, false, true, 3) MCE_F16_INST(2, false, true, 3) MCE_F16_INST(3, false, true, 3) MCE_F16_INST(4, false, true, 3)
#define MCE_F16_INST32(KST) template __global__ void knn_f16_kernel<KST, 32, false, false, 1>(const _Float16*, int64_t, int, const _Float16*, const double*, const double*, const double*, const double*, int64_t, int64_t, int, int64_t, int, int, int64_t, int, double*, int*, const int*, const float*, int, const int*, const int*, const float*, const float*, const float*, int, int, const int*, const double*, const int*, int, SymParams, float*);
MCE_F16_INST32(1) MCE_F16_INST32(2) MCE_F16_INST32(3) MCE_F16_INST32(4)
#endif
#if MCE_KCAP == 4
template __global__ void knn_f16_kernel<1, MCE_KCAP, false, false, 0, MCE_KCAP, 4>(const _Float16*, int64_t, int, const _Float16*, const double*, const double*, const double*, const double*, int64_t, int64_t, int, int64_t, int, int, int64_t, int, double*, int*, const int*, const float*, int, const int*, const int*, const float*, const float*, const float*, int, int, const int*, const double*, const int*, int, SymParams, float*);
#endif
#endif
#if MCE_INST_PANEL
template __global__ void knn_panel_kernel<1, MCE_KCAP>(PanelArgs);
template __global__ void knn_panel_kernel<2, MCE_KCAP>(PanelArgs);
template __global__ void knn_panel_kernel<3, MCE_KCAP>(PanelArgs);
template __global__ void knn_panel_kernel<4, MCE_KCAP>(PanelArgs);
#if MCE_KCAP == 16
template __global__ void knn_panel_kernel<1, MCE_KCAP, true>(PanelArgs);
template __global__ void knn_panel_kernel<2, MCE_KCAP, true>(PanelArgs);
template __global__ void knn_panel_kernel<3, MCE_KCAP, true>(PanelArgs);
template __global__ void knn_panel_kernel<4, MCE_KCAP, true>(PanelArgs);
#endif
#endif
#if MCE_INST_F64
#define MCE_INST(KS) template __global__ void knn_mfma_kernel<KS, MCE_KCAP>(const double*, int64_t, int, const double*, const double*, int64_t, int, int64_t, int, int, int64_t, int, double*, int*);
MCE_INST(1) MCE_INST(2) MCE_INST(3) MCE_INST(4) MCE_INST(5) MCE_INST(6) MCE_INST(7) MCE_INST(8)
MCE_INST(9) MCE_INST(10) MCE_INST(11) MCE_INST(12) MCE_INST(13) MCE_INST(14) MCE_INST(15) MCE_INST(16)
MCE_INST(20) MCE_INST(24) MCE_INST(28) MCE_INST(32)
#endif
#endif

}
```

### mcevidence_amd/csrc/knn_panel.hpp

```cpp
#pragma once
#include "knn_f16.hpp"

namespace mce {

struct PanelArgs {
    const _Float16* Yh;
    const _Float16* Xh;
    const double* qinfo;
    const double* params;
    const double* X;
    const double* Y;
    const int* rperm;
    double* part_d;
    int* part_i;
    int64_t nq, nr, nq_pad, self_offset;
    int D, ksel, self_exclude, spin_limit;
    int debug;
    SymParams sym;
    PanelGeom geom;
    const PanelUnit* units = nullptr;
    const double* lo_d = nullptr;
    const int* lo_i = nullptr;
};

#ifndef MCE_PANEL_STATS
#define MCE_PANEL_STATS 0
#endif
#ifndef MCE_PANEL_NPASS
#define MCE_PANEL_NPASS 3
#endif
#ifndef MCE_PANEL_STAGE_KB
#define MCE_PANEL_STAGE_KB MCE_H_STAGE_KB
#endif
#ifndef MCE_PANEL_QUEUE
#define MCE_PANEL_QUEUE MCE_H_QUEUE
#endif
#ifndef MCE_PANEL_TRIGGER
#define MCE_PANEL_TRIGGER 192
#endif
#ifndef MCE_PANEL_ABL
#define MCE_PANEL_ABL 0
#endif

__host__ __device__ constexpr int panel_chunk_tiles(int KST) { return MCE_PANEL_STAGE_KB / KST / 2 * 2; }
constexpr int kPanelQueue = MCE_PANEL_QUEUE;
__host__ __device__ constexpr size_t panel_lds_bytes(int KST)
{
    return (size_t)2 * panel_chunk_tiles(KST) * KST * 1024
           + (size_t)kHWaves * kPanelQueue * 16
           + (size_t)kHWaves * kHQT * 32 * 4 + 128
           + (size_t)kHWaves * kHQT * 32 * 4
           + (size_t)kHWaves * panel_chunk_tiles(KST) * kHQT * 4;
}

template <class T> __device__ __forceinline__ const __attribute__((address_space(1))) T* gptr(const T* p)
{
    return (const __attribute__((address_space(1))) T*)p;
}
template <class T> __device__ __forceinline__ __attribute__((address_space(1))) T* gptr_w(T* p)
{
    return (__attribute__((address_space(1))) T*)p;
}

__device__ __forceinline__ float vmaxf(float a, float b)
{
    float r;
    asm("v_max_f32 %0, %1, %2" : "=v"(r) : "v"(a), "v"(b));
    return r;
}

template <int KST, int KCAP, bool LOWER = false>
__global__ __launch_bounds__(kHThreads, 2) void knn_panel_kernel(PanelArgs args_by_value)
{
    static_assert(kHQT == 2 && kHNL == 1, "8 waves x 2 query tiles, one list per owner lane");
    constexpr int QT = 2;
    constexpr int QPW = 64;
    constexpr int QPB = kHWaves * QPW;
    constexpr int TPB = QPB / 32;
    constexpr int CT = panel_chunk_tiles(KST);
    constexpr int CHUNK_BYTES = CT * KST * 1024;
    constexpr int VPT = CHUNK_BYTES / 16 / kHThreads;
    static_assert(CHUNK_BYTES % (16 * kHThreads) == 0 && CT % 2 == 0, "chunk geometry");
    constexpr int QN = kPanelQueue;
    (void)args_by_value;
    typedef const __attribute__((address_space(4))) PanelArgs* ArgsPtr;
    const ArgsPtr ap0 = (ArgsPtr)__builtin_amdgcn_kernarg_segment_ptr();
#define MCE_ARGS() ([&]() __attribute__((always_inline)) { ArgsPtr p_ = ap0; asm volatile("" : "+s"(p_)); return p_; }())

    extern __shared__ __attribute__((aligned(16))) char lds_raw[];
    char* const stage0 = lds_raw;
    double* const qd2_all = reinterpret_cast<double*>(lds_raw + 2 * CHUNK_BYTES);
    int* const qpk_all = reinterpret_cast<int*>(qd2_all + kHWaves * QN);
    int* const qnx_all = qpk_all + kHWaves * QN;
    int* const head_all = qnx_all + kHWaves * QN;
    volatile int* const wvote = head_all + kHWaves * QPW;
    float* const sthr_all = reinterpret_cast<float*>(head_all + kHWaves * QPW + 32);
    int* const redo_all = reinterpret_cast<int*>(sthr_all + kHWaves * QPW);

    const int tid = threadIdx.x;
    const int lane = tid & 63;
    const int wave = __builtin_amdgcn_readfirstlane(tid >> 6);
    double* const wqd = qd2_all + wave * QN;
    int* const wq = qpk_all + wave * QN;
    int* const wnx = qnx_all + wave * QN;
    int* const whead = head_all + wave * QPW;
    float* const sthr = sthr_all + wave * QPW;
    int* const wredo = redo_all + wave * (CT * QT);
    const double INF = __builtin_huge_val();

#if MCE_PANEL_STATS
    const long long t_kernel0 = clock64();
    long long st_drains = 0, st_enq = 0, st_events = 0, st_redo = 0, st_tD = 0, st_tE = 0, st_tPro = 0, st_tA = 0, st_tR = 0, st_tB = 0;
#endif

    int sym_p, qblk, t_lo, t_hi, useq, sym_on, qb_lo;
    {
        const ArgsPtr a = MCE_ARGS();
        if (a->units) {
            const auto u = (const __attribute__((address_space(1))) PanelUnit*)a->units + blockIdx.x;
            qblk = __builtin_amdgcn_readfirstlane(u->qblk);
            t_lo = __builtin_amdgcn_readfirstlane(u->t_lo);
            t_hi = __builtin_amdgcn_readfirstlane(u->t_hi);
            useq = __builtin_amdgcn_readfirstlane(u->useq);
            sym_p = 0;
            sym_on = a->geom.sym_on;
            qb_lo = a->geom.qb_lo;
        } else {
            PanelGeom g;
            g.qb_lo = a->geom.qb_lo; g.qb_hi = a->geom.qb_hi; g.tpb = a->geom.tpb; g.tpp = a->geom.tpp;
            g.ct = a->geom.ct; g.ntiles = a->geom.ntiles; g.sym_on = a->geom.sym_on;
            panel_unit_decode((int)blockIdx.x, g, sym_p, qblk);
            panel_unit_tiles(sym_p, qblk, g, t_lo, t_hi);
            useq = panel_unit_seq(sym_p, qblk, g);
            sym_on = g.sym_on;
            qb_lo = g.qb_lo;
        }
    }
    auto chain_of = [&](int& chain, int64_t& list_off) __attribute__((always_inline)) {
        const ArgsPtr a = MCE_ARGS();
        chain = qblk;
        list_off = 0;
        if (a->units) {
            const auto u = (const __attribute__((address_space(1))) PanelUnit*)a->units + blockIdx.x;
            chain = __builtin_amdgcn_readfirstlane(u->chain);
            list_off = (int64_t)__builtin_amdgcn_readfirstlane(u->list_set) * KCAP * a->nq_pad;
        }
    };
    const int64_t qwave0 = (int64_t)qblk * QPB + wave * QPW;

    whead[lane] = -1;
    if (tid < 3) wvote[tid] = 0;

    double own_d[KCAP];
    int own_i[KCAP];
#pragma unroll
    for (int k = 0; k < KCAP; ++k) { own_d[k] = INF; own_i[k] = -1; }
    double seed_thr = INF;

    {
        const ArgsPtr a = MCE_ARGS();
        if (useq > 0) {
            int chain;
            int64_t list_off;
            chain_of(chain, list_off);
            int spins = 0;
            const int limit = ((a->debug & 16) && useq == 1 && (wave & 1)) ? -1 : a->spin_limit;
            bool ok = true;
            const auto done = gptr(a->sym.done);
            while (spins > limit || __hip_atomic_load(done + chain, __ATOMIC_RELAXED, __HIP_MEMORY_SCOPE_AGENT) < useq) {
                if (++spins > limit) { ok = false; break; }
                __builtin_amdgcn_s_sleep(32);
            }
            __builtin_amdgcn_fence(__ATOMIC_ACQUIRE, "agent");
            if (ok && gptr(a->sym.bucket_flag)[qblk] != 0) ok = false;
            if (ok) {
                const int64_t q = qwave0 + lane;
                const int64_t np = a->nq_pad;
                const auto pd = gptr(a->part_d) + list_off;
                const auto pi = gptr(a->part_i) + list_off;
#pragma unroll
                for (int k = 0; k < KCAP; ++k) {
                    own_d[k] = pd[(int64_t)k * np + q];
                    own_i[k] = pi[(int64_t)k * np + q];
                }
            } else if (lane == 0) {
                gptr_w(a->sym.bucket_flag)[qblk] = 1;
            }
        }
    }

    v8h b[QT][KST];
    float G[QT], cR[QT];
    unsigned lanew[QT];
    const int k_last = MCE_ARGS()->ksel - 1;
    {
        const ArgsPtr a = MCE_ARGS();
        const auto Xh = gptr(a->Xh);
#pragma unroll
        for (int qt = 0; qt < QT; ++qt) {
            const int64_t q = qwave0 + qt * 32 + (lane & 31);
#pragma unroll
            for (int ks = 0; ks < KST; ++ks)
                b[qt][ks] = *(const __attribute__((address_space(1))) v8h*)(Xh + q * (int64_t)(16 * KST) + 16 * ks + 8 * (lane >> 5));
            lanew[qt] = ((unsigned)(qt * 32 + (lane & 31)) << kHRelBits) | (unsigned)(4 * (lane >> 5));
            cR[qt] = -__builtin_huge_valf();
            G[qt] = -__builtin_huge_valf();
        }
    }
    double gq_a[QT], gq_c[QT], own_a = 0.0, s2c, rowc;
    {
        const ArgsPtr a = MCE_ARGS();
        const auto params = gptr(a->params);
        const auto qinfo = gptr(a->qinfo);
        const double p_scale = params[HP_SCALE], p_ey = params[HP_EY], p_ym = params[HP_YHATMAX], p_rho = params[HP_RHO];
        s2c = p_scale * p_scale;
        rowc = f16_row_const(p_ym);
#pragma unroll
        for (int qt = 0; qt < QT; ++qt) {
            const int64_t q = qwave0 + qt * 32 + (lane & 31);
            gq_a[qt] = 0.0;
            gq_c[qt] = -INF;
            if (q < a->nq && MCE_PANEL_ABL != 1) {
                const F16GateTerms t = f16_gate_terms(qinfo[2 * q], qinfo[2 * q + 1], p_ey, p_ym, p_rho, KST);
                gq_a[qt] = t.a;
                gq_c[qt] = t.c;
            }
        }
        {
            const int64_t q = qwave0 + lane;
            if (q < a->nq) own_a = f16_gate_a(qinfo[2 * q], p_ey, KST);
        }
    }
    auto gate_of = [&](double thr, int qt) __attribute__((always_inline)) -> float { return f16_gate(thr, s2c, gq_a[qt], gq_c[qt]); };
    auto own_row_gate = [&](double thr) __attribute__((always_inline)) -> float { return f16_row_gate(thr, s2c, own_a, rowc); };
    {
        const ArgsPtr a = MCE_ARGS();
        const int64_t q = qwave0 + lane;
        double t0 = INF;
        if (sym_on) t0 = __longlong_as_double((long long)__hip_atomic_load(gptr(a->sym.thr) + q, __ATOMIC_RELAXED, __HIP_MEMORY_SCOPE_AGENT));
        else if (a->sym.thr) t0 = __longlong_as_double((long long)gptr(a->sym.thr)[q]);
        seed_thr = t0;
        double tl = own_d[KCAP - 1];
#pragma unroll
        for (int k = 0; k < KCAP - 1; ++k) tl = (k == k_last) ? own_d[k] : tl;
        t0 = fmin(t0, tl);
        sthr[lane] = __double2float_ru(t0);
#pragma unroll
        for (int qt = 0; qt < QT; ++qt) G[qt] = gate_of(__shfl(t0, qt * 32 + (lane & 31), 64), qt);
        if (sym_on) {
#pragma unroll
            for (int qt = 0; qt < QT; ++qt) cR[qt] = gq_c[qt] > -INF ? f16_round_up(gq_c[qt]) : -__builtin_huge_valf();
        }
    }

    const int dbg_flags = MCE_ARGS()->debug;
    const int qlimit_gate = (dbg_flags & 8) ? -1 : QN - 64;
    int qcount = 0;
    int nredo = 0;

    auto drain = [&]() __attribute__((always_inline)) {
#if MCE_PANEL_STATS
        const long long t_d0 = clock64();
        st_drains += 1; st_enq += qcount;
#endif
        const ArgsPtr a = MCE_ARGS();
        const auto X = gptr(a->X);
        const auto Y = gptr(a->Y);
        const int D = a->D;
        const int64_t nq = a->nq, nr = a->nr;
        const int self_exclude = a->self_exclude;
        const int64_t self_offset = a->self_offset;
        const auto rperm = gptr(a->rperm);
        {
            const int sub = lane & 7;
            constexpr int NPASS = KST > 2 ? 1 : MCE_PANEL_NPASS;
            constexpr int EPL = KST > 2 ? 8 : 4;
            for (int b0 = 0; b0 < qcount; b0 += NPASS * 8) {
                int qlp[NPASS], ep[NPASS];
                bool okp[NPASS];
                const __attribute__((address_space(1))) double* xp[NPASS];
                const __attribute__((address_space(1))) double* yp[NPASS];
#pragma unroll
                for (int u = 0; u < NPASS; ++u) {
                    const int e = b0 + u * 8 + (lane >> 3);
                    ep[u] = e;
                    int ql = 0, j = 0;
                    const bool valid = e < qcount;
                    if (valid) {
                        const unsigned ent = (unsigned)wq[e];
                        ql = (int)(ent >> kHRelBits);
                        j = (int)(ent & ((1u << kHSymRowBits) - 1u));
                    }
                    qlp[u] = ql;
                    const int64_t q = qwave0 + ql;
                    okp[u] = valid && j < nr && q < nq && !(self_exclude && (int64_t)j == self_offset + q);
                    xp[u] = X + (okp[u] ? q : 0) * (int64_t)D;
                    yp[u] = Y + (okp[u] ? (int64_t)j : 0) * D;
                }
                double xv[NPASS][EPL], yv[NPASS][EPL];
#pragma unroll
                for (int u = 0; u < NPASS; ++u)
#pragma unroll
                    for (int v = 0; v < EPL; ++v) {
                        const int iv = (sub + 8 * v < D) ? sub + 8 * v : (sub < D ? sub : D - 1);
                        xv[u][v] = xp[u][iv];
                        yv[u][v] = yp[u][iv];
                    }
#pragma unroll
                for (int u = 0; u < NPASS; ++u) {
                    double a0 = 0.0;
#pragma unroll
                    for (int v = 0; v < EPL; ++v) {
                        const double t = (sub + 8 * v < D) ? xv[u][v] - yv[u][v] : 0.0;
                        a0 = fma(t, t, a0);
                    }
                    a0 += __shfl_xor(a0, 1, 64);
                    a0 += __shfl_xor(a0, 2, 64);
                    a0 += __shfl_xor(a0, 4, 64);
                    if (sub == 0 && ep[u] < qcount) {
                        wqd[ep[u]] = okp[u] ? a0 : -1.0;
                        bool col = okp[u] && !(a0 > (double)sthr[qlp[u]]);
                        if constexpr (LOWER) {
                            if (col) {
                                const int64_t o = (int64_t)(KCAP - 1) * a->nq_pad + qwave0 + qlp[u];
                                const double ld = gptr(a->lo_d)[o];
                                const int li = gptr(a->lo_i)[o];
                                const int jr = (int)((unsigned)wq[ep[u]] & ((1u << kHSymRowBits) - 1u));
                                const int jc = rperm ? rperm[jr] : jr;
                                col = a0 > ld || (a0 == ld && jc > li);
                            }
                        }
                        if (col) wnx[ep[u]] = atomicExch(&whead[qlp[u]], ep[u]);
                    }
                }
            }
        }
        __builtin_amdgcn_fence(__ATOMIC_ACQ_REL, "wavefront");
#if MCE_PANEL_STATS
        const long long t_dA = clock64();
        st_tA += t_dA - t_d0;
#endif
        {
            const auto sp_thr = gptr_w(a->sym.thr);
            const auto sp_rrow = gptr_w(a->sym.rrow);
            const auto sp_rtile = gptr_w(a->sym.rtile);
            const auto sp_slots = gptr_w(a->sym.slots);
            const auto sp_bucket_cnt = gptr_w(a->sym.bucket_cnt);
            const auto sp_bucket_flag = gptr_w(a->sym.bucket_flag);
            const auto sp_bucket = gptr_w(a->sym.bucket);
            const int sp_cap = a->sym.cap;
            const int ksel = a->ksel;
            auto row_gate = [&](double thr, int row) { return f16_row_gate_of(thr, gptr(a->qinfo)[2 * (int64_t)row], a->params, KST); };
            for (int e0 = 0; e0 < qcount; e0 += 64) {
                const int e = e0 + lane;
                const bool valid = e < qcount;
                const unsigned ent = valid ? (unsigned)wq[e] : 0u;
                const int ql = (int)(ent >> kHRelBits);
                const int j = (int)(ent & ((1u << kHSymRowBits) - 1u));
                const bool rowflag = (ent >> kHSymRowBits) & 1u;
                const double d2 = valid ? wqd[e] : -1.0;
                const bool ok = valid && d2 >= 0.0;
                const int oj = ok ? (rperm ? rperm[j] : j) : -1;
                bool rs = ok && rowflag;
                if (rs) {
                    const int jb = j / QPB;
                    rs = d2 <= __longlong_as_double((long long)__hip_atomic_load(sp_thr + j, __ATOMIC_RELAXED, __HIP_MEMORY_SCOPE_AGENT));
                    if constexpr (LOWER) {
                        if (rs) {
                            const int64_t o = (int64_t)(KCAP - 1) * a->nq_pad + j;
                            const double ld = gptr(a->lo_d)[o];
                            const int li = gptr(a->lo_i)[o];
                            const int sc = rperm ? rperm[qwave0 + ql] : (int)(qwave0 + ql);
                            rs = d2 > ld || (d2 == ld && sc > li);
                        }
                    }
                    if (rs) rs = sym_slot_insert<KCAP>(sp_slots, sp_thr, sp_rrow, sp_rtile, ksel, j, d2, row_gate);
                    if (rs) {
                        const int slot = __hip_atomic_fetch_add(sp_bucket_cnt + jb, 1, __ATOMIC_RELAXED, __HIP_MEMORY_SCOPE_AGENT);
                        if ((unsigned)slot < (unsigned)sp_cap) {
                            const auto en = sp_bucket + ((int64_t)jb * sp_cap + slot);
                            en->d2 = d2;
                            en->src = rperm ? rperm[qwave0 + ql] : (int)(qwave0 + ql);
                            en->row = j;
                        } else {
                            sp_bucket_flag[jb] = 1;
                        }
                    }
                }
                if (valid) wq[e] = oj;
            }
        }
        __builtin_amdgcn_fence(__ATOMIC_ACQ_REL, "wavefront");
#if MCE_PANEL_STATS
        const long long t_dR = clock64();
        st_tR += t_dR - t_dA;
#endif
        {
            int cur = whead[lane];
            whead[lane] = -1;
            while (__any(cur >= 0)) {
                const bool on = cur >= 0;
                const int ce = on ? cur : 0;
                const double d2 = on ? wqd[ce] : INF;
                const int j = wq[ce];
                cur = on ? wnx[ce] : -1;
                list_insert<KCAP>(own_d, own_i, d2, j);
            }
        }
        qcount = 0;
        double thr_own = own_d[KCAP - 1];
#pragma unroll
        for (int k = 0; k < KCAP - 1; ++k) thr_own = (k == k_last) ? own_d[k] : thr_own;
        thr_own = fmin(thr_own, seed_thr);
        if (sym_on) {
            const auto sp_thr = gptr_w(a->sym.thr);
            const auto sp_rrow = gptr_w(a->sym.rrow);
            const auto sp_rtile = gptr_w(a->sym.rtile);
            const int64_t q = qwave0 + lane;
            double t = thr_own;
            float R = 0.0f;
            if (q < nq) {
                if (t < INF) {
                    const unsigned long long mb = (unsigned long long)__double_as_longlong(t);
                    const unsigned rb = __float_as_uint(own_row_gate(t));
                    const unsigned long long ob = __hip_atomic_fetch_min(sp_thr + q, mb, __ATOMIC_RELAXED, __HIP_MEMORY_SCOPE_AGENT);
                    const unsigned orb = __hip_atomic_fetch_min(sp_rrow + q, rb, __ATOMIC_RELAXED, __HIP_MEMORY_SCOPE_AGENT);
                    t = fmin(t, __longlong_as_double((long long)ob));
                    R = __uint_as_float(rb < orb ? rb : orb);
                } else {
                    t = __longlong_as_double((long long)__hip_atomic_load(sp_thr + q, __ATOMIC_RELAXED, __HIP_MEMORY_SCOPE_AGENT));
                    const unsigned rb = __float_as_uint(own_row_gate(t));
                    const unsigned orb = __hip_atomic_fetch_min(sp_rrow + q, rb, __ATOMIC_RELAXED, __HIP_MEMORY_SCOPE_AGENT);
                    R = __uint_as_float(rb < orb ? rb : orb);
                }
            }
            thr_own = t;
            seed_thr = t;
            float m = R;
#pragma unroll
            for (int o = 16; o >= 1; o >>= 1) m = fmaxf(m, __shfl_xor(m, o, 64));
            if ((lane & 31) == 0) __hip_atomic_store(sp_rtile + ((qwave0 + lane) >> 5), m, __ATOMIC_RELAXED, __HIP_MEMORY_SCOPE_AGENT);
        }
        sthr[lane] = __double2float_ru(thr_own);
#pragma unroll
        for (int qt = 0; qt < QT; ++qt) G[qt] = gate_of(__shfl(thr_own, qt * 32 + (lane & 31), 64), qt);
#if MCE_PANEL_STATS
        st_tD += clock64() - t_d0;
#endif
    };

    auto event = [&](const v16f& c, const float (&l1)[5], const int qt, const float gq, const bool rowflag, const int jb0, const unsigned todo, const int qlimit) __attribute__((always_inline)) -> unsigned {
        return f16_event<true>(c, l1, lanew[qt], gq, rowflag, jb0, todo, qlimit, wq, qcount);
    };

    const auto Yh_bytes = (const __attribute__((address_space(1))) char*)MCE_ARGS()->Yh;
    auto stage_async = [&](int64_t c, int buf) { f16_stage_chunk<VPT>(Yh_bytes + c * (int64_t)CHUNK_BYTES, stage0 + buf * CHUNK_BYTES, tid, wave); };
    auto load_a = [&](const char* lp, v8h (&a)[KST]) { f16_load_a<KST>(lp, a); };
    auto mfma_first = [&](const v8h (&a)[KST], v16f (&acc)[QT]) __attribute__((always_inline)) {
#pragma unroll
        for (int qt = 0; qt < QT; ++qt) {
            v16f z = {0.f, 0.f, 0.f, 0.f, 0.f, 0.f, 0.f, 0.f, 0.f, 0.f, 0.f, 0.f, 0.f, 0.f, 0.f, 0.f};
            acc[qt] = __builtin_amdgcn_mfma_f32_32x32x16_f16(a[0], b[qt][0], z, 0, 0, 0);
        }
    };
    auto mfma_rest = [&](const v8h (&a)[KST], v16f (&acc)[QT]) __attribute__((always_inline)) {
#pragma unroll
        for (int ks = 1; ks < KST; ++ks)
#pragma unroll
            for (int qt = 0; qt < QT; ++qt) acc[qt] = __builtin_amdgcn_mfma_f32_32x32x16_f16(a[ks], b[qt][ks], acc[qt], 0, 0, 0);
    };
#if defined(__HIP_DEVICE_COMPILE__)
#define MCE_ORDER(GATED_, NEXT_) asm volatile("" : "+v"(GATED_[0]), "+v"(GATED_[1]), "+v"(NEXT_[0]), "+v"(NEXT_[1]))
#else
#define MCE_ORDER(GATED_, NEXT_) do {} while (0)
#endif
    auto gate_tile = [&](const v16f (&acc)[QT], const int jb0, const float (&gq)[QT], const float (&rg)[QT], const int tix) __attribute__((always_inline)) {
#if MCE_PANEL_ABL == 2
#if defined(__HIP_DEVICE_COMPILE__)
        asm volatile("" :: "v"(acc[0]), "v"(acc[1]));
#endif
        return;
#endif
        float l1[QT][5], mm[QT];
        bool pq[QT];
#pragma unroll
        for (int qt = 0; qt < QT; ++qt) {
            mm[qt] = f16_min16(acc[qt], l1[qt]);
            pq[qt] = mm[qt] <= gq[qt];
        }
        if (__any(pq[0] || pq[1])) {
#pragma unroll
            for (int qt = 0; qt < QT; ++qt) {
                if (!__any(pq[qt])) continue;
#if MCE_PANEL_STATS
                st_events += 1;
                const long long t_e0 = clock64();
#endif
                const unsigned rem = event(acc[qt], l1[qt], qt, gq[qt], mm[qt] <= rg[qt], jb0, 0xffffu, qlimit_gate);
                if (rem) {
                    if (lane == 0) wredo[nredo] = (int)(rem | ((unsigned)qt << 16) | ((unsigned)tix << 17));
                    nredo += 1;
                }
#if MCE_PANEL_STATS
                st_tE += clock64() - t_e0;
#endif
            }
        }
    };

    const int cfirst = t_lo / CT;
    const int ntot = (t_hi - 1) / CT - cfirst + 1;
    const auto rtile_p = gptr(MCE_ARGS()->sym.rtile);
    auto rt_load = [&](int c) -> float {
        const int t = c * CT + lane;
        const int tb = t / TPB;
        const bool en = sym_on && lane < CT && tb >= qb_lo && tb < qblk && MCE_PANEL_ABL != 1;
        const float r = en ? __hip_atomic_load(rtile_p + t, __ATOMIC_RELAXED, __HIP_MEMORY_SCOPE_AGENT) : -__builtin_huge_valf();
        return fmaxf(r, __shfl_xor(r, 1, 64));
    };
    float rt_cur = -__builtin_huge_valf(), rt_next;
    stage_async(cfirst, 0);
    rt_next = rt_load(cfirst);
#if MCE_PANEL_STATS
    st_tPro = clock64() - t_kernel0;
#endif
    v16f accA[QT], accB[QT];
    for (int k = 0; k < ntot; ++k) {
        const int buf = k & 1;
        const int c = cfirst + k;
        const int vs = k % 3;
        if (qcount >= MCE_PANEL_TRIGGER && lane == 0) wvote[vs] = 1;
#if MCE_PANEL_STATS
        const long long t_b0 = clock64();
#endif
        dma_barrier();
#if MCE_PANEL_STATS
        st_tB += clock64() - t_b0;
#endif
        if (tid == 0) wvote[vs == 0 ? 2 : vs - 1] = 0;
        rt_cur = rt_next;
        if (k + 1 < ntot) {
            stage_async(c + 1, buf ^ 1);
            rt_next = rt_load(c + 1);
        }
        bool need_drain = __builtin_amdgcn_readfirstlane(wvote[vs]) != 0 || k + 1 == ntot;
        const int tlo = (k == 0) ? t_lo - c * CT : 0;
        const int thi = t_hi - c * CT < CT ? t_hi - c * CT : CT;
        const char* const lbuf = stage0 + buf * CHUNK_BYTES + lane * 16;
        const int jchunk = c * (CT * 32);
        {
            v8h a0[KST], a1[KST];
            load_a(lbuf + (tlo * KST) * 1024, a0);
            load_a(lbuf + ((tlo + 1) * KST) * 1024, a1);
            mfma_first(a0, accA);
            mfma_rest(a0, accA);
            int t = tlo;
            float gqP[QT], rgP[QT];
            _Pragma("unroll 1") for (;;)
            {
                const float rP = __uint_as_float((unsigned)__builtin_amdgcn_readlane((int)__float_as_uint(rt_cur), t));
#pragma unroll
                for (int qt = 0; qt < QT; ++qt) {
                    rgP[qt] = rP + cR[qt];
                    gqP[qt] = vmaxf(G[qt], rgP[qt]);
                }
                const bool more = t + 2 < thi;
                load_a(lbuf + ((more ? t + 2 : t) * KST) * 1024, a0);
                mfma_first(a1, accB);
                MCE_ORDER(accA, accB);
                mfma_rest(a1, accB);
                gate_tile(accA, jchunk + t * 32, gqP, rgP, t);
                if (!more) break;
                load_a(lbuf + ((t + 3) * KST) * 1024, a1);
                mfma_first(a0, accA);
                MCE_ORDER(accB, accA);
                mfma_rest(a0, accA);
                gate_tile(accB, jchunk + (t + 1) * 32, gqP, rgP, t + 1);
                t += 2;
            }
            {
#if defined(__HIP_DEVICE_COMPILE__)
                asm volatile("s_nop 15\n\ts_nop 3" : "+v"(accB[0]), "+v"(accB[1]));
#endif
                gate_tile(accB, jchunk + (t + 1) * 32, gqP, rgP, t + 1);
            }
        }
        while (need_drain || nredo > 0 || (k + 1 == ntot && qcount > 0)) {
            drain();
            need_drain = false;
            const int n = nredo;
            nredo = 0;
            for (int i = 0; i < n; ++i) {
                const unsigned w = (unsigned)__builtin_amdgcn_readfirstlane(wredo[i]);
                const unsigned todo = w & 0xffffu;
                const int qt = (int)((w >> 16) & 1u), t = (int)(w >> 17);
                const float Rt = __uint_as_float((unsigned)__builtin_amdgcn_readlane((int)__float_as_uint(rt_cur), t));
                v8h at[KST];
                load_a(lbuf + (t * KST) * 1024, at);
                v16f z = {0.f, 0.f, 0.f, 0.f, 0.f, 0.f, 0.f, 0.f, 0.f, 0.f, 0.f, 0.f, 0.f, 0.f, 0.f, 0.f};
                v16f r_ = z;
                if (qt == 0) {
#pragma unroll
                    for (int ks = 0; ks < KST; ++ks) r_ = __builtin_amdgcn_mfma_f32_32x32x16_f16(at[ks], b[0][ks], r_, 0, 0, 0);
                } else {
#pragma unroll
                    for (int ks = 0; ks < KST; ++ks) r_ = __builtin_amdgcn_mfma_f32_32x32x16_f16(at[ks], b[1][ks], r_, 0, 0, 0);
                }
#if defined(__HIP_DEVICE_COMPILE__)
                asm volatile("s_nop 15\n\ts_nop 3" : "+v"(r_));
#endif
                float l1[5];
                const float mm = f16_min16(r_, l1);
                const float rg = Rt + (qt ? cR[1] : cR[0]);
                const float gq = vmaxf(qt ? G[1] : G[0], rg);
                unsigned rem = 0;
                if (__any(mm <= gq)) rem = event(r_, l1, qt, gq, mm <= rg, jchunk + t * 32, todo, QN - 64);
                if (rem) {
                    if (lane == 0) wredo[nredo] = (int)(rem | ((unsigned)qt << 16) | ((unsigned)t << 17));
                    nredo += 1;
                }
#if MCE_PANEL_STATS
                st_redo += 1;
#endif
            }
        }
    }

#if MCE_PANEL_STATS
    if (lane == 0) {
        const ArgsPtr a = MCE_ARGS();
        double* o = const_cast<double*>(a->params) + 16 + ((int64_t)blockIdx.x * kHWaves + wave) * 8;
        o[0] = (double)st_drains; o[1] = (double)st_enq; o[2] = (double)st_redo; o[3] = (double)st_events;
        o[4] = (double)st_tE; o[5] = (double)st_tD; o[6] = (double)(clock64() - t_kernel0); o[7] = (double)st_tPro;
        double* o2 = const_cast<double*>(a->params) + 16 + ((int64_t)gridDim.x * kHWaves) * 8 + ((int64_t)blockIdx.x * kHWaves + wave) * 8;
        o2[0] = (double)st_tA; o2[1] = (double)st_tR; o2[2] = (double)(st_tD - st_tA - st_tR); o2[3] = (double)st_tB; o2[4] = 0; o2[5] = 0; o2[6] = 0; o2[7] = 0;
    }
#endif
    {
        const ArgsPtr a = MCE_ARGS();
        const int64_t q = qwave0 + lane;
        const int64_t np = a->nq_pad;
        int chain;
        int64_t list_off;
        chain_of(chain, list_off);
        const auto pd = gptr_w(a->part_d) + list_off;
        const auto pi = gptr_w(a->part_i) + list_off;
#pragma unroll
        for (int k = 0; k < KCAP; ++k) {
            pd[(int64_t)k * np + q] = own_d[k];
            pi[(int64_t)k * np + q] = own_i[k];
        }
        __builtin_amdgcn_fence(__ATOMIC_RELEASE, "agent");
        __syncthreads();
        if (tid == 0) __hip_atomic_fetch_add(gptr_w(a->sym.done) + chain, 1, __ATOMIC_RELAXED, __HIP_MEMORY_SCOPE_AGENT);
    }
#undef MCE_ARGS
}

}
```

Before: 26.81 million.

## Add wide panel kernel with four query tiles per wave for large symmetric searches

Adds a QT=4 variant of the symmetric panel kernel in which each wave handles 128 queries. Staged data-row tiles are reused across twice as many query tiles, roughly halving LDS staging traffic per query. To limit register pressure, the per-query candidate lists stay in global memory rather than registers. The wide kernel is picked automatically when nq==nr and there are enough query blocks, and it can be forced on or off through MCE_PANEL_QT. The costs are extra global memory traffic for the lists, a smaller event queue, and fewer query blocks to spread across CUs.

```diff
diff --git a/mcevidence_amd/csrc/capi_common.hpp b/mcevidence_amd/csrc/capi_common.hpp
--- a/mcevidence_amd/csrc/capi_common.hpp
+++ b/mcevidence_amd/csrc/capi_common.hpp
@@ -35,7 +35,7 @@
 struct Tuning {
     bool sym_kernel_f16 = false, tail_split = true, prune_prof = false, wide = true;
     int spin_limit = 1 << 21, sym_bucket = 0, sym_panel = 0, sym_seed_rows = 0, sym_seed_share = 2, sym_seed_mode = -1;
-    int f16_seed_rows = -1, f16_seed_share = -1, f16_seed_tg = -1, rsplit = 0, panel_debug = 0, sym_chains = 0;
+    int f16_seed_rows = -1, f16_seed_share = -1, f16_seed_tg = -1, rsplit = 0, panel_debug = 0, sym_chains = 0, panel_qt = 0;
     size_t feed_wave_bytes = 0;
 };
 Tuning read_tuning()
@@ -58,6 +58,7 @@
     t.tail_split = num("MCE_TAIL_SPLIT", 1) != 0;
     t.wide = num("MCE_WIDE", 1) != 0;
     t.panel_debug = num("MCE_PANEL_DEBUG", 0);
+    t.panel_qt = num("MCE_PANEL_QT", 0);
     t.prune_prof = getenv("MCE_PRUNE_PROF") != nullptr;
     if ((e = getenv("MCE_FEED_WAVE_BYTES"))) t.feed_wave_bytes = (size_t)std::strtoull(e, nullptr, 10);
     return t;
diff --git a/mcevidence_amd/csrc/capi_plan.hpp b/mcevidence_amd/csrc/capi_plan.hpp
--- a/mcevidence_amd/csrc/capi_plan.hpp
+++ b/mcevidence_amd/csrc/capi_plan.hpp
@@ -11,6 +11,7 @@
 constexpr double kPruneHeavyFullRounds = 10.0;
 constexpr int kPruneHeavySplit = 4, kPruneHeavyMaxSplit = 8;
 constexpr int kPruneWaveQueries = mce::kHQT * 32;
+constexpr int kPanelWideMinBlocks = 1954;
 constexpr int kWideMinBlocks = 480;
 bool prune_heavy_enabled()
 {
@@ -42,6 +43,7 @@
     double cost = 0.0;
     int ksel = 0;
     bool twopass = false;
+    bool panel_wide_ok = false;
     bool wide_ok = false;
     bool prune = false;
     bool kd_ready = false;
@@ -221,10 +223,12 @@
     p.nqblk = (int)std::max<int64_t>(1, (nq + qpb - 1) / qpb);
     p.wide_ok = f16 && !p.twopass && p.KST == 1 && p.vh->launch_wide && p.nqblk >= kWideMinBlocks && nr <= ((int64_t)1 << 25) && read_tuning().wide;
     if (p.wide_ok && (p.nqblk & 1)) p.nqblk += 1;
+    const bool panel_wide_shape = f16 && !p.twopass && nq == nr && p.vh->launch_panel_wide && p.vh->launch_sym && p.nqblk >= 2;
     p.nq_pad = (int64_t)p.nqblk * qpb;
     const int64_t rows_per_chunk = (int64_t)p.CT * rows_per_tile;
     p.nchunk = (nr + rows_per_chunk - 1) / rows_per_chunk;
     p.nrow_pad = p.nchunk * rows_per_chunk;
+    p.panel_wide_ok = panel_wide_shape && p.nrow_pad <= ((int64_t)1 << (mce::kHSymRowBits - 1));
 
     if (f16 && !p.twopass && p.KST == 1 && d <= mce::kPruneMaxDim && p.vh->launch_prune && nq > 0 &&
         p.nrow_pad <= ((int64_t)1 << mce::kHRelBits) && (int64_t)p.nqblk * p.nchunk <= mce::kPruneMaxPairs) {
diff --git a/mcevidence_amd/csrc/capi_search.hpp b/mcevidence_amd/csrc/capi_search.hpp
--- a/mcevidence_amd/csrc/capi_search.hpp
+++ b/mcevidence_amd/csrc/capi_search.hpp
@@ -329,8 +329,10 @@
 {
     int units = mce::sym_unit_count(p.nqblk, mce::kHWaves * mce::kHQT, panel * p.CT, (int)((nr + 31) / 32) + (int)(((nr + 31) / 32) & 1));
     double tiles = 0.0;
+    double qtiles = 16.0;
     if (panel_kernel) {
         units = mce::panel_unit_count(g);
+        qtiles = g.tpb;
         for (int u = 0; g_prof_on && u < units; ++u) {
             int pp, aa, lo, hi;
             mce::panel_unit_decode(u, g, pp, aa);
@@ -341,7 +343,7 @@
         const double tpb = mce::kHWaves * mce::kHQT, T = (double)((nr + 31) / 32);
         for (int b = 0; b < p.nqblk; ++b) tiles += std::min(tpb * (b + 1), T);
     }
-    g_last_flops_main = tiles * 16.0 * 1024.0 * 32.0 * p.KST;
+    g_last_flops_main = tiles * qtiles * 1024.0 * 32.0 * p.KST;
     return units;
 }
 
@@ -383,6 +385,9 @@
         }
     }
     const bool unit_table = apo || geom.nsplit > 1;
+    const bool panel_wide = panel_kernel && p.panel_wide_ok && p.nparts == 1 && !p.twopass && !unit_table &&
+                            (tun.panel_qt == 4 || (tun.panel_qt != 2 && p.nqblk >= kPanelWideMinBlocks));
+    if (panel_wide) { geom.tpb = 2 * mce::kHWaves * mce::kHQT; geom.qb_lo = 0; geom.qb_hi = (p.nqblk + 1) / 2; }
     const int npass = p.twopass ? 2 : 1;
     int seed_used = 0;
     for (int pass = 0; pass < npass; ++pass) {
@@ -427,7 +432,7 @@
                 }
                 pa.units = tab;
             }
-            MCE_HIP((lower ? p.vh->launch_panel_lower : p.vh->launch_panel)(pa, st));
+            MCE_HIP((lower ? p.vh->launch_panel_lower : (panel_wide ? p.vh->launch_panel_wide : p.vh->launch_panel))(pa, st));
         } else {
             MCE_HIP(p.vh->launch_sym(a, st));
         }
@@ -446,7 +451,7 @@
     g_last_flops_all = g_last_flops_main + (double)(seed_used & 0xffff) * p.CT * (double)(qb_hi - qb_lo) * 16.0 * 1024.0 * 32.0 * p.KST;
     snprintf(g_last_kernel, sizeof(g_last_kernel), "%s symmetric%s%s%s grid=%d block=%d lds=%zu qt=%d ct=%d panel=%d seed=%dx%d/%d bucket=%d", p.vh->name, panel_kernel ? " panel-kernel" : "",
              p.twopass ? " two passes" : "", geom.blk_stride > 1 ? " pairs-once" : (geom.nsplit > 1 ? " chains" : ""), sym_units,
-             mce::kHThreads, panel_kernel ? p.vh->lds_bytes_panel : p.vh->lds_bytes_sym, p.QT, p.CT, a.sym.panel, seed_used & 0xffff, (seed_used >> 16) & 0xfff, (seed_used >> 28) & 3, p.sl.cap);
+             mce::kHThreads, panel_wide ? p.vh->lds_bytes_panel_wide : (panel_kernel ? p.vh->lds_bytes_panel : p.vh->lds_bytes_sym), panel_wide ? 2 * p.QT : p.QT, p.CT, a.sym.panel, seed_used & 0xffff, (seed_used >> 16) & 0xfff, (seed_used >> 28) & 3, p.sl.cap);
     return MCE_OK;
 }
 
diff --git a/mcevidence_amd/csrc/f16_filter.hpp b/mcevidence_amd/csrc/f16_filter.hpp
--- a/mcevidence_amd/csrc/f16_filter.hpp
+++ b/mcevidence_amd/csrc/f16_filter.hpp
@@ -166,11 +166,11 @@
     }
 }
 
-template <bool ROWFLAG>
+template <bool ROWFLAG, int ROWBIT = kHSymRowBits>
 __device__ __forceinline__ unsigned f16_event(const v16f& c, const float (&l1)[5], const unsigned lanew, const float g, const bool rowflag, const int jb0,
                                               const unsigned todo, const int qlimit, int* const wq, int& qcount)
 {
-    const unsigned wbase = (lanew + (unsigned)jb0) | (ROWFLAG && rowflag ? (1u << kHSymRowBits) : 0u);
+    const unsigned wbase = (lanew + (unsigned)jb0) | (ROWFLAG && rowflag ? (1u << ROWBIT) : 0u);
     unsigned rem = 0;
 #define MCE_HIT(R_, P_, S_)                                                                                               \
     if ((S_) != 0 && (todo & (1u << (R_)))) {                                                                             \
diff --git a/mcevidence_amd/csrc/knn_dispatch.hpp b/mcevidence_amd/csrc/knn_dispatch.hpp
--- a/mcevidence_amd/csrc/knn_dispatch.hpp
+++ b/mcevidence_amd/csrc/knn_dispatch.hpp
@@ -93,6 +93,8 @@
     knn_panel_launch_fn launch_panel_lower;
     knn_f16_launch_fn launch_sym_repair_lower;
     knn_f16_launch_fn launch_sym_pre32;
+    knn_panel_launch_fn launch_panel_wide;
+    size_t lds_bytes_panel_wide;
 };
 struct DeepArgs;
 typedef hipError_t (*knn_deep_launch_fn)(const DeepArgs&, hipStream_t);
diff --git a/mcevidence_amd/csrc/knn_inst.hip b/mcevidence_amd/csrc/knn_inst.hip
--- a/mcevidence_amd/csrc/knn_inst.hip
+++ b/mcevidence_amd/csrc/knn_inst.hip
@@ -69,14 +69,14 @@
 #endif
 
 #if MCE_INST_F16 || MCE_INST_PANEL
-template <int KST, int KCAP, bool LOWER = false>
+template <int KST, int KCAP, bool LOWER = false, int QT = 2>
 hipError_t launch_panel_variant(const PanelArgs& a, hipStream_t st)
 #if MCE_INST_PANEL
 {
-    constexpr size_t LDS = panel_lds_bytes(KST);
+    constexpr size_t LDS = panel_lds_bytes(KST, QT);
     static_assert(LDS <= 160 * 1024, "LDS budget");
     static bool attr_set[kMaxDevices] = {};
-    auto kern = knn_panel_kernel<KST, KCAP, LOWER>;
+    auto kern = knn_panel_kernel<KST, KCAP, LOWER, QT>;
     int dev = 0;
     (void)hipGetDevice(&dev);
     if (dev >= kMaxDevices || !attr_set[dev]) {
@@ -84,6 +84,7 @@
         if (e != hipSuccess) return e;
         if (dev < kMaxDevices) attr_set[dev] = true;
     }
+    if (a.geom.tpb != 8 * QT) return hipErrorInvalidValue;
     const int units = panel_unit_count(a.geom);
     if (units <= 0) return hipSuccess;
     hipLaunchKernelGGL(kern, dim3((unsigned)units), dim3(kHThreads), LDS, st, a);
@@ -93,6 +94,8 @@
 template hipError_t launch_panel_variant<2, MCE_KCAP>(const PanelArgs&, hipStream_t);
 template hipError_t launch_panel_variant<3, MCE_KCAP>(const PanelArgs&, hipStream_t);
 template hipError_t launch_panel_variant<4, MCE_KCAP>(const PanelArgs&, hipStream_t);
+template hipError_t launch_panel_variant<1, MCE_KCAP, false, 4>(const PanelArgs&, hipStream_t);
+template hipError_t launch_panel_variant<2, MCE_KCAP, false, 4>(const PanelArgs&, hipStream_t);
 #if MCE_KCAP == 16
 template hipError_t launch_panel_variant<1, MCE_KCAP, true>(const PanelArgs&, hipStream_t);
 template hipError_t launch_panel_variant<2, MCE_KCAP, true>(const PanelArgs&, hipStream_t);
@@ -105,6 +108,8 @@
 extern template hipError_t launch_panel_variant<2, MCE_KCAP>(const PanelArgs&, hipStream_t);
 extern template hipError_t launch_panel_variant<3, MCE_KCAP>(const PanelArgs&, hipStream_t);
 extern template hipError_t launch_panel_variant<4, MCE_KCAP>(const PanelArgs&, hipStream_t);
+extern template hipError_t launch_panel_variant<1, MCE_KCAP, false, 4>(const PanelArgs&, hipStream_t);
+extern template hipError_t launch_panel_variant<2, MCE_KCAP, false, 4>(const PanelArgs&, hipStream_t);
 #if MCE_KCAP == 16
 extern template hipError_t launch_panel_variant<1, MCE_KCAP, true>(const PanelArgs&, hipStream_t);
 extern template hipError_t launch_panel_variant<2, MCE_KCAP, true>(const PanelArgs&, hipStream_t);
@@ -171,11 +176,12 @@
 #else
 #define MCE_F16_WIDE(KST) nullptr, 0
 #endif
+#define MCE_PANEL_WIDE(KST) ((KST) <= 2 ? &launch_panel_variant<((KST) <= 2 ? (KST) : 2), MCE_KCAP, false, 4> : (knn_panel_launch_fn) nullptr), ((KST) <= 2 ? panel_lds_bytes(KST, 4) : 0)
 #define MCE_F16_VARIANT(KST, PRUNE_FN)                                                                   \
     {&launch_f16_variant<KST, MCE_KCAP, false>, PRUNE_FN, MCE_F16_LOWER(KST), &launch_f16_variant<KST, MCE_KCAP, false, false, 1>, \
      &launch_f16_variant<KST, MCE_KCAP, false, false, 2>, &launch_f16_variant<KST, MCE_KCAP, false, false, 3>, &launch_panel_variant<KST, MCE_KCAP>, panel_lds_bytes(KST), \
      f16_lds_bytes(KST, MCE_KCAP, true), KST, MCE_KCAP, f16_qt(MCE_KCAP), f16_chunk_tiles(KST), \
-     f16_lds_bytes(KST, MCE_KCAP), "knn_f16_kernel<KST=" #KST ",KCAP=" MCE_STR(MCE_KCAP) ">", MCE_F16_SHORT(KST), MCE_F16_WIDE(KST), MCE_F16_SYM_LOWER(KST)}
+     f16_lds_bytes(KST, MCE_KCAP), "knn_f16_kernel<KST=" #KST ",KCAP=" MCE_STR(MCE_KCAP) ">", MCE_F16_SHORT(KST), MCE_F16_WIDE(KST), MCE_F16_SYM_LOWER(KST), MCE_PANEL_WIDE(KST)}
 extern const KnnF16Variant MCE_CAT(g_knn_f16_kcap, MCE_KCAP)[kMaxKST] = {
     MCE_F16_VARIANT(1, (&launch_f16_variant<1, MCE_KCAP, true>)), MCE_F16_VARIANT(2, nullptr), MCE_F16_VARIANT(3, nullptr),
     MCE_F16_VARIANT(4, nullptr),
@@ -226,6 +232,8 @@
 template __global__ void knn_panel_kernel<2, MCE_KCAP>(PanelArgs);
 template __global__ void knn_panel_kernel<3, MCE_KCAP>(PanelArgs);
 template __global__ void knn_panel_kernel<4, MCE_KCAP>(PanelArgs);
+template __global__ void knn_panel_kernel<1, MCE_KCAP, false, 4>(PanelArgs);
+template __global__ void knn_panel_kernel<2, MCE_KCAP, false, 4>(PanelArgs);
 #if MCE_KCAP == 16
 template __global__ void knn_panel_kernel<1, MCE_KCAP, true>(PanelArgs);
 template __global__ void knn_panel_kernel<2, MCE_KCAP, true>(PanelArgs);
diff --git a/mcevidence_amd/csrc/knn_panel.hpp b/mcevidence_amd/csrc/knn_panel.hpp
--- a/mcevidence_amd/csrc/knn_panel.hpp
+++ b/mcevidence_amd/csrc/knn_panel.hpp
@@ -44,13 +44,14 @@
 
 __host__ __device__ constexpr int panel_chunk_tiles(int KST) { return MCE_PANEL_STAGE_KB / KST / 2 * 2; }
 constexpr int kPanelQueue = MCE_PANEL_QUEUE;
-__host__ __device__ constexpr size_t panel_lds_bytes(int KST)
+__host__ __device__ constexpr int panel_queue(int QT) { return QT == 4 ? (kPanelQueue < 384 ? kPanelQueue : 384) : kPanelQueue; }
+__host__ __device__ constexpr size_t panel_lds_bytes(int KST, int QT = kHQT)
 {
     return (size_t)2 * panel_chunk_tiles(KST) * KST * 1024
-           + (size_t)kHWaves * kPanelQueue * 16
-           + (size_t)kHWaves * kHQT * 32 * 4 + 128
-           + (size_t)kHWaves * kHQT * 32 * 4
-           + (size_t)kHWaves * panel_chunk_tiles(KST) * kHQT * 4;
+           + (size_t)kHWaves * panel_queue(QT) * 16
+           + (size_t)kHWaves * QT * 32 * 4 + 128
+           + (size_t)kHWaves * QT * 32 * 4
+           + (size_t)kHWaves * panel_chunk_tiles(KST) * QT * 4;
 }
 
 template <class T> __device__ __forceinline__ const __attribute__((address_space(1))) T* gptr(const T* p)
@@ -69,19 +70,23 @@
     return r;
 }
 
-template <int KST, int KCAP, bool LOWER = false>
+constexpr int kPanelPlanRows = kHWaves * 64;
+template <int KST, int KCAP, bool LOWER = false, int QT = 2>
 __global__ __launch_bounds__(kHThreads, 2) void knn_panel_kernel(PanelArgs args_by_value)
 {
-    static_assert(kHQT == 2 && kHNL == 1, "8 waves x 2 query tiles, one list per owner lane");
-    constexpr int QT = 2;
-    constexpr int QPW = 64;
+    static_assert(QT == 2 || QT == 4, "two or four query tiles per wave");
+    constexpr int NL = QT / 2;
+    constexpr int QPW = 32 * QT;
     constexpr int QPB = kHWaves * QPW;
+    constexpr int PBW = QPB / kPanelPlanRows;
     constexpr int TPB = QPB / 32;
+    constexpr int RELB = QT == 4 ? 25 : kHRelBits;
+    constexpr int ROWB = RELB - 1;
     constexpr int CT = panel_chunk_tiles(KST);
     constexpr int CHUNK_BYTES = CT * KST * 1024;
     constexpr int VPT = CHUNK_BYTES / 16 / kHThreads;
     static_assert(CHUNK_BYTES % (16 * kHThreads) == 0 && CT % 2 == 0, "chunk geometry");
-    constexpr int QN = kPanelQueue;
+    constexpr int QN = panel_queue(QT);
     (void)args_by_value;
     typedef const __attribute__((address_space(4))) PanelArgs* ArgsPtr;
     const ArgsPtr ap0 = (ArgsPtr)__builtin_amdgcn_kernarg_segment_ptr();
@@ -147,15 +152,25 @@
         }
     };
     const int64_t qwave0 = (int64_t)qblk * QPB + wave * QPW;
-
-    whead[lane] = -1;
+    const bool wave_live = PBW == 1 || qwave0 < MCE_ARGS()->nq_pad;
+
+#pragma unroll
+    for (int nl = 0; nl < NL; ++nl) whead[nl * 64 + lane] = -1;
     if (tid < 3) wvote[tid] = 0;
 
-    double own_d[KCAP];
-    int own_i[KCAP];
-#pragma unroll
-    for (int k = 0; k < KCAP; ++k) { own_d[k] = INF; own_i[k] = -1; }
-    double seed_thr = INF;
+    constexpr bool LMEM = QT == 4;
+    bool list_in_mem = false, trusted = true;
+    double reg_d[NL][KCAP];
+    int reg_i[NL][KCAP];
+    if constexpr (!LMEM) {
+#pragma unroll
+        for (int k = 0; k < KCAP; ++k) { reg_d[0][k] = INF; reg_i[0][k] = -1; }
+    }
+    const int k_last = MCE_ARGS()->ksel - 1;
+    double list_kth[NL];
+    double seed_thr[NL];
+#pragma unroll
+    for (int nl = 0; nl < NL; ++nl) { list_kth[nl] = INF; seed_thr[nl] = INF; }
 
     {
         const ArgsPtr a = MCE_ARGS();
@@ -172,19 +187,28 @@
                 __builtin_amdgcn_s_sleep(32);
             }
             __builtin_amdgcn_fence(__ATOMIC_ACQUIRE, "agent");
-            if (ok && gptr(a->sym.bucket_flag)[qblk] != 0) ok = false;
+#pragma unroll
+            for (int h = 0; h < PBW; ++h)
+                if (ok && (PBW == 1 || (int64_t)(qblk * PBW + h) * kPanelPlanRows < a->nq_pad) && gptr(a->sym.bucket_flag)[qblk * PBW + h] != 0) ok = false;
+            ok = __builtin_amdgcn_readfirstlane((int)ok) != 0;
             if (ok) {
-                const int64_t q = qwave0 + lane;
-                const int64_t np = a->nq_pad;
-                const auto pd = gptr(a->part_d) + list_off;
-                const auto pi = gptr(a->part_i) + list_off;
-#pragma unroll
-                for (int k = 0; k < KCAP; ++k) {
-                    own_d[k] = pd[(int64_t)k * np + q];
-                    own_i[k] = pi[(int64_t)k * np + q];
-                }
-            } else if (lane == 0) {
-                gptr_w(a->sym.bucket_flag)[qblk] = 1;
+                list_in_mem = true;
+                if constexpr (!LMEM) {
+                    const int64_t q = qwave0 + lane;
+                    const int64_t np = a->nq_pad;
+                    const auto pd = gptr(a->part_d) + list_off;
+                    const auto pi = gptr(a->part_i) + list_off;
+#pragma unroll
+                    for (int k = 0; k < KCAP; ++k) {
+                        reg_d[0][k] = pd[(int64_t)k * np + q];
+                        reg_i[0][k] = pi[(int64_t)k * np + q];
+                    }
+                }
+#pragma unroll
+                for (int nl = 0; nl < NL; ++nl) list_kth[nl] = (!LMEM || !wave_live) ? INF : (gptr(a->part_d) + list_off)[(int64_t)k_last * a->nq_pad + qwave0 + nl * 64 + lane];
+            } else {
+                trusted = false;
+                if (lane < PBW && (PBW == 1 || (int64_t)(qblk * PBW + lane) * kPanelPlanRows < a->nq_pad)) gptr_w(a->sym.bucket_flag)[qblk * PBW + lane] = 1;
             }
         }
     }
@@ -192,7 +216,6 @@
     v8h b[QT][KST];
     float G[QT], cR[QT];
     unsigned lanew[QT];
-    const int k_last = MCE_ARGS()->ksel - 1;
     {
         const ArgsPtr a = MCE_ARGS();
         const auto Xh = gptr(a->Xh);
@@ -200,14 +223,16 @@
         for (int qt = 0; qt < QT; ++qt) {
             const int64_t q = qwave0 + qt * 32 + (lane & 31);
 #pragma unroll
-            for (int ks = 0; ks < KST; ++ks)
-                b[qt][ks] = *(const __attribute__((address_space(1))) v8h*)(Xh + q * (int64_t)(16 * KST) + 16 * ks + 8 * (lane >> 5));
-            lanew[qt] = ((unsigned)(qt * 32 + (lane & 31)) << kHRelBits) | (unsigned)(4 * (lane >> 5));
+            for (int ks = 0; ks < KST; ++ks) {
+                const v8h zero = {0, 0, 0, 0, 0, 0, 0, 0};
+                b[qt][ks] = wave_live ? *(const __attribute__((address_space(1))) v8h*)(Xh + q * (int64_t)(16 * KST) + 16 * ks + 8 * (lane >> 5)) : zero;
+            }
+            lanew[qt] = ((unsigned)(qt * 32 + (lane & 31)) << RELB) | (unsigned)(4 * (lane >> 5));
             cR[qt] = -__builtin_huge_valf();
             G[qt] = -__builtin_huge_valf();
         }
     }
-    double gq_a[QT], gq_c[QT], own_a = 0.0, s2c, rowc;
+    double gq_a[QT], gq_c[QT], own_a[NL], s2c, rowc;
     {
         const ArgsPtr a = MCE_ARGS();
         const auto params = gptr(a->params);
@@ -226,27 +251,37 @@
                 gq_c[qt] = t.c;
             }
         }
-        {
-            const int64_t q = qwave0 + lane;
-            if (q < a->nq) own_a = f16_gate_a(qinfo[2 * q], p_ey, KST);
+#pragma unroll
+        for (int nl = 0; nl < NL; ++nl) {
+            const int64_t q = qwave0 + nl * 64 + lane;
+            own_a[nl] = 0.0;
+            if (q < a->nq) own_a[nl] = f16_gate_a(qinfo[2 * q], p_ey, KST);
         }
     }
     auto gate_of = [&](double thr, int qt) __attribute__((always_inline)) -> float { return f16_gate(thr, s2c, gq_a[qt], gq_c[qt]); };
-    auto own_row_gate = [&](double thr) __attribute__((always_inline)) -> float { return f16_row_gate(thr, s2c, own_a, rowc); };
+    auto own_row_gate = [&](double thr, int nl) __attribute__((always_inline)) -> float { return f16_row_gate(thr, s2c, own_a[nl], rowc); };
     {
         const ArgsPtr a = MCE_ARGS();
-        const int64_t q = qwave0 + lane;
-        double t0 = INF;
-        if (sym_on) t0 = __longlong_as_double((long long)__hip_atomic_load(gptr(a->sym.thr) + q, __ATOMIC_RELAXED, __HIP_MEMORY_SCOPE_AGENT));
-        else if (a->sym.thr) t0 = __longlong_as_double((long long)gptr(a->sym.thr)[q]);
-        seed_thr = t0;
-        double tl = own_d[KCAP - 1];
-#pragma unroll
-        for (int k = 0; k < KCAP - 1; ++k) tl = (k == k_last) ? own_d[k] : tl;
-        t0 = fmin(t0, tl);
-        sthr[lane] = __double2float_ru(t0);
-#pragma unroll
-        for (int qt = 0; qt < QT; ++qt) G[qt] = gate_of(__shfl(t0, qt * 32 + (lane & 31), 64), qt);
+        double t0[NL];
+#pragma unroll
+        for (int nl = 0; nl < NL; ++nl) {
+            const int64_t q = qwave0 + nl * 64 + lane;
+            t0[nl] = INF;
+            if (!wave_live) t0[nl] = INF;
+            else if (sym_on) t0[nl] = __longlong_as_double((long long)__hip_atomic_load(gptr(a->sym.thr) + q, __ATOMIC_RELAXED, __HIP_MEMORY_SCOPE_AGENT));
+            else if (a->sym.thr) t0[nl] = __longlong_as_double((long long)gptr(a->sym.thr)[q]);
+            seed_thr[nl] = t0[nl];
+            if constexpr (!LMEM) {
+                double tl = reg_d[0][KCAP - 1];
+#pragma unroll
+                for (int k = 0; k < KCAP - 1; ++k) tl = (k == k_last) ? reg_d[0][k] : tl;
+                list_kth[nl] = tl;
+            }
+            t0[nl] = fmin(t0[nl], list_kth[nl]);
+            sthr[nl * 64 + lane] = __double2float_ru(t0[nl]);
+        }
+#pragma unroll
+        for (int qt = 0; qt < QT; ++qt) G[qt] = gate_of(__shfl(t0[qt / 2], (qt & 1) * 32 + (lane & 31), 64), qt);
         if (sym_on) {
 #pragma unroll
             for (int qt = 0; qt < QT; ++qt) cR[qt] = gq_c[qt] > -INF ? f16_round_up(gq_c[qt]) : -__builtin_huge_valf();
@@ -271,6 +306,31 @@
         const int self_exclude = a->self_exclude;
         const int64_t self_offset = a->self_offset;
         const auto rperm = gptr(a->rperm);
+        double loc_d[NL][KCAP];
+        int loc_i[NL][KCAP];
+        double (&own_d)[NL][KCAP] = *(LMEM ? &loc_d : &reg_d);
+        int (&own_i)[NL][KCAP] = *(LMEM ? &loc_i : &reg_i);
+        int chain_;
+        int64_t list_off;
+        chain_of(chain_, list_off);
+        const int64_t own_o = list_off + qwave0 + lane;
+        const int64_t npad = a->nq_pad;
+        auto list_load = [&](const int nl) __attribute__((always_inline)) {
+            if constexpr (!LMEM) return;
+            if (list_in_mem && wave_live) {
+                const auto pd = (const __attribute__((address_space(1))) unsigned long long*)(a->part_d) + own_o + nl * 64;
+                const auto pi = gptr(a->part_i) + own_o + nl * 64;
+#pragma unroll
+                for (int k = 0; k < KCAP; ++k) {
+                    own_d[nl][k] = __longlong_as_double((long long)__hip_atomic_load(pd + (int64_t)k * npad, __ATOMIC_RELAXED, __HIP_MEMORY_SCOPE_AGENT));
+                    own_i[nl][k] = __hip_atomic_load(pi + (int64_t)k * npad, __ATOMIC_RELAXED, __HIP_MEMORY_SCOPE_AGENT);
+                }
+            } else {
+#pragma unroll
+                for (int k = 0; k < KCAP; ++k) { own_d[nl][k] = INF; own_i[nl][k] = -1; }
+            }
+        };
+        list_load(0);
         {
             const int sub = lane & 7;
             constexpr int NPASS = KST > 2 ? 1 : MCE_PANEL_NPASS;
@@ -288,8 +348,8 @@
                     const bool valid = e < qcount;
                     if (valid) {
                         const unsigned ent = (unsigned)wq[e];
-                        ql = (int)(ent >> kHRelBits);
-                        j = (int)(ent & ((1u << kHSymRowBits) - 1u));
+                        ql = (int)(ent >> RELB);
+                        j = (int)(ent & ((1u << ROWB) - 1u));
                     }
                     qlp[u] = ql;
                     const int64_t q = qwave0 + ql;
@@ -325,7 +385,7 @@
                                 const int64_t o = (int64_t)(KCAP - 1) * a->nq_pad + qwave0 + qlp[u];
                                 const double ld = gptr(a->lo_d)[o];
                                 const int li = gptr(a->lo_i)[o];
-                                const int jr = (int)((unsigned)wq[ep[u]] & ((1u << kHSymRowBits) - 1u));
+                                const int jr = (int)((unsigned)wq[ep[u]] & ((1u << ROWB) - 1u));
                                 const int jc = rperm ? rperm[jr] : jr;
                                 col = a0 > ld || (a0 == ld && jc > li);
                             }
@@ -355,15 +415,15 @@
                 const int e = e0 + lane;
                 const bool valid = e < qcount;
                 const unsigned ent = valid ? (unsigned)wq[e] : 0u;
-                const int ql = (int)(ent >> kHRelBits);
-                const int j = (int)(ent & ((1u << kHSymRowBits) - 1u));
-                const bool rowflag = (ent >> kHSymRowBits) & 1u;
+                const int ql = (int)(ent >> RELB);
+                const int j = (int)(ent & ((1u << ROWB) - 1u));
+                const bool rowflag = (ent >> ROWB) & 1u;
                 const double d2 = valid ? wqd[e] : -1.0;
                 const bool ok = valid && d2 >= 0.0;
                 const int oj = ok ? (rperm ? rperm[j] : j) : -1;
                 bool rs = ok && rowflag;
                 if (rs) {
-                    const int jb = j / QPB;
+                    const int jb = j / kPanelPlanRows;
                     rs = d2 <= __longlong_as_double((long long)__hip_atomic_load(sp_thr + j, __ATOMIC_RELAXED, __HIP_MEMORY_SCOPE_AGENT));
                     if constexpr (LOWER) {
                         if (rs) {
@@ -395,110 +455,128 @@
         const long long t_dR = clock64();
         st_tR += t_dR - t_dA;
 #endif
-        {
-            int cur = whead[lane];
-            whead[lane] = -1;
+        double thr_own[NL];
+#pragma unroll
+        for (int nl = 0; nl < NL; ++nl) {
+            if (nl + 1 < NL) list_load(nl + 1);
+            int cur = whead[nl * 64 + lane];
+            whead[nl * 64 + lane] = -1;
             while (__any(cur >= 0)) {
                 const bool on = cur >= 0;
                 const int ce = on ? cur : 0;
                 const double d2 = on ? wqd[ce] : INF;
                 const int j = wq[ce];
                 cur = on ? wnx[ce] : -1;
-                list_insert<KCAP>(own_d, own_i, d2, j);
-            }
-        }
+                list_insert<KCAP>(own_d[nl], own_i[nl], d2, j);
+            }
+            if (LMEM && trusted && wave_live) {
+                const auto pd = gptr_w(a->part_d) + own_o + nl * 64;
+                const auto pi = gptr_w(a->part_i) + own_o + nl * 64;
+#pragma unroll
+                for (int k = 0; k < KCAP; ++k) {
+                    pd[(int64_t)k * npad] = own_d[nl][k];
+                    pi[(int64_t)k * npad] = own_i[nl][k];
+                }
+            }
+            double t = own_d[nl][KCAP - 1];
+#pragma unroll
+            for (int k = 0; k < KCAP - 1; ++k) t = (k == k_last) ? own_d[nl][k] : t;
+            thr_own[nl] = fmin(t, seed_thr[nl]);
+            seed_thr[nl] = thr_own[nl];
+        }
+        if (trusted) list_in_mem = true;
         qcount = 0;
-        double thr_own = own_d[KCAP - 1];
-#pragma unroll
-        for (int k = 0; k < KCAP - 1; ++k) thr_own = (k == k_last) ? own_d[k] : thr_own;
-        thr_own = fmin(thr_own, seed_thr);
         if (sym_on) {
             const auto sp_thr = gptr_w(a->sym.thr);
             const auto sp_rrow = gptr_w(a->sym.rrow);
             const auto sp_rtile = gptr_w(a->sym.rtile);
-            const int64_t q = qwave0 + lane;
-            double t = thr_own;
-            float R = 0.0f;
-            if (q < nq) {
-                if (t < INF) {
-                    const unsigned long long mb = (unsigned long long)__double_as_longlong(t);
-                    const unsigned rb = __float_as_uint(own_row_gate(t));
-                    const unsigned long long ob = __hip_atomic_fetch_min(sp_thr + q, mb, __ATOMIC_RELAXED, __HIP_MEMORY_SCOPE_AGENT);
-                    const unsigned orb = __hip_atomic_fetch_min(sp_rrow + q, rb, __ATOMIC_RELAXED, __HIP_MEMORY_SCOPE_AGENT);
-                    t = fmin(t, __longlong_as_double((long long)ob));
-                    R = __uint_as_float(rb < orb ? rb : orb);
-                } else {
-                    t = __longlong_as_double((long long)__hip_atomic_load(sp_thr + q, __ATOMIC_RELAXED, __HIP_MEMORY_SCOPE_AGENT));
-                    const unsigned rb = __float_as_uint(own_row_gate(t));
-                    const unsigned orb = __hip_atomic_fetch_min(sp_rrow + q, rb, __ATOMIC_RELAXED, __HIP_MEMORY_SCOPE_AGENT);
-                    R = __uint_as_float(rb < orb ? rb : orb);
-                }
-            }
-            thr_own = t;
-            seed_thr = t;
-            float m = R;
-#pragma unroll
-            for (int o = 16; o >= 1; o >>= 1) m = fmaxf(m, __shfl_xor(m, o, 64));
-            if ((lane & 31) == 0) __hip_atomic_store(sp_rtile + ((qwave0 + lane) >> 5), m, __ATOMIC_RELAXED, __HIP_MEMORY_SCOPE_AGENT);
-        }
-        sthr[lane] = __double2float_ru(thr_own);
-#pragma unroll
-        for (int qt = 0; qt < QT; ++qt) G[qt] = gate_of(__shfl(thr_own, qt * 32 + (lane & 31), 64), qt);
+#pragma unroll
+            for (int nl = 0; nl < NL; ++nl) {
+                const int64_t q = qwave0 + nl * 64 + lane;
+                double t = thr_own[nl];
+                float R = 0.0f;
+                if (q < nq) {
+                    if (t < INF) {
+                        const unsigned long long mb = (unsigned long long)__double_as_longlong(t);
+                        const unsigned rb = __float_as_uint(own_row_gate(t, nl));
+                        const unsigned long long ob = __hip_atomic_fetch_min(sp_thr + q, mb, __ATOMIC_RELAXED, __HIP_MEMORY_SCOPE_AGENT);
+                        const unsigned orb = __hip_atomic_fetch_min(sp_rrow + q, rb, __ATOMIC_RELAXED, __HIP_MEMORY_SCOPE_AGENT);
+                        t = fmin(t, __longlong_as_double((long long)ob));
+                        R = __uint_as_float(rb < orb ? rb : orb);
+                    } else {
+                        t = __longlong_as_double((long long)__hip_atomic_load(sp_thr + q, __ATOMIC_RELAXED, __HIP_MEMORY_SCOPE_AGENT));
+                        const unsigned rb = __float_as_uint(own_row_gate(t, nl));
+                        const unsigned orb = __hip_atomic_fetch_min(sp_rrow + q, rb, __ATOMIC_RELAXED, __HIP_MEMORY_SCOPE_AGENT);
+                        R = __uint_as_float(rb < orb ? rb : orb);
+                    }
+                }
+                thr_own[nl] = t;
+                seed_thr[nl] = t;
+                float m = R;
+#pragma unroll
+                for (int o = 16; o >= 1; o >>= 1) m = fmaxf(m, __shfl_xor(m, o, 64));
+                if ((lane & 31) == 0 && wave_live) __hip_atomic_store(sp_rtile + ((qwave0 + nl * 64 + lane) >> 5), m, __ATOMIC_RELAXED, __HIP_MEMORY_SCOPE_AGENT);
+            }
+        }
+#pragma unroll
+        for (int nl = 0; nl < NL; ++nl) sthr[nl * 64 + lane] = __double2float_ru(thr_own[nl]);
+#pragma unroll
+        for (int qt = 0; qt < QT; ++qt) G[qt] = gate_of(__shfl(thr_own[qt / 2], (qt & 1) * 32 + (lane & 31), 64), qt);
 #if MCE_PANEL_STATS
         st_tD += clock64() - t_d0;
 #endif
     };
 
     auto event = [&](const v16f& c, const float (&l1)[5], const int qt, const float gq, const bool rowflag, const int jb0, const unsigned todo, const int qlimit) __attribute__((always_inline)) -> unsigned {
-        return f16_event<true>(c, l1, lanew[qt], gq, rowflag, jb0, todo, qlimit, wq, qcount);
+        return f16_event<true, ROWB>(c, l1, lanew[qt], gq, rowflag, jb0, todo, qlimit, wq, qcount);
     };
 
     const auto Yh_bytes = (const __attribute__((address_space(1))) char*)MCE_ARGS()->Yh;
     auto stage_async = [&](int64_t c, int buf) { f16_stage_chunk<VPT>(Yh_bytes + c * (int64_t)CHUNK_BYTES, stage0 + buf * CHUNK_BYTES, tid, wave); };
     auto load_a = [&](const char* lp, v8h (&a)[KST]) { f16_load_a<KST>(lp, a); };
-    auto mfma_first = [&](const v8h (&a)[KST], v16f (&acc)[QT]) __attribute__((always_inline)) {
-#pragma unroll
-        for (int qt = 0; qt < QT; ++qt) {
+    auto mfma_first = [&](const v8h (&a)[KST], v16f (&acc)[2], const int q0) __attribute__((always_inline)) {
+#pragma unroll
+        for (int qt = 0; qt < 2; ++qt) {
             v16f z = {0.f, 0.f, 0.f, 0.f, 0.f, 0.f, 0.f, 0.f, 0.f, 0.f, 0.f, 0.f, 0.f, 0.f, 0.f, 0.f};
-            acc[qt] = __builtin_amdgcn_mfma_f32_32x32x16_f16(a[0], b[qt][0], z, 0, 0, 0);
+            acc[qt] = __builtin_amdgcn_mfma_f32_32x32x16_f16(a[0], b[q0 + qt][0], z, 0, 0, 0);
         }
     };
-    auto mfma_rest = [&](const v8h (&a)[KST], v16f (&acc)[QT]) __attribute__((always_inline)) {
+    auto mfma_rest = [&](const v8h (&a)[KST], v16f (&acc)[2], const int q0) __attribute__((always_inline)) {
 #pragma unroll
         for (int ks = 1; ks < KST; ++ks)
 #pragma unroll
-            for (int qt = 0; qt < QT; ++qt) acc[qt] = __builtin_amdgcn_mfma_f32_32x32x16_f16(a[ks], b[qt][ks], acc[qt], 0, 0, 0);
+            for (int qt = 0; qt < 2; ++qt) acc[qt] = __builtin_amdgcn_mfma_f32_32x32x16_f16(a[ks], b[q0 + qt][ks], acc[qt], 0, 0, 0);
     };
 #if defined(__HIP_DEVICE_COMPILE__)
 #define MCE_ORDER(GATED_, NEXT_) asm volatile("" : "+v"(GATED_[0]), "+v"(GATED_[1]), "+v"(NEXT_[0]), "+v"(NEXT_[1]))
 #else
 #define MCE_ORDER(GATED_, NEXT_) do {} while (0)
 #endif
-    auto gate_tile = [&](const v16f (&acc)[QT], const int jb0, const float (&gq)[QT], const float (&rg)[QT], const int tix) __attribute__((always_inline)) {
+    auto gate_tile = [&](const v16f (&acc)[2], const int jb0, const float (&gq)[QT], const float (&rg)[QT], const int tix, const int q0) __attribute__((always_inline)) {
 #if MCE_PANEL_ABL == 2
 #if defined(__HIP_DEVICE_COMPILE__)
         asm volatile("" :: "v"(acc[0]), "v"(acc[1]));
 #endif
         return;
 #endif
-        float l1[QT][5], mm[QT];
-        bool pq[QT];
-#pragma unroll
-        for (int qt = 0; qt < QT; ++qt) {
+        float l1[2][5], mm[2];
+        bool pq[2];
+#pragma unroll
+        for (int qt = 0; qt < 2; ++qt) {
             mm[qt] = f16_min16(acc[qt], l1[qt]);
-            pq[qt] = mm[qt] <= gq[qt];
+            pq[qt] = mm[qt] <= gq[q0 + qt];
         }
         if (__any(pq[0] || pq[1])) {
 #pragma unroll
-            for (int qt = 0; qt < QT; ++qt) {
+            for (int qt = 0; qt < 2; ++qt) {
                 if (!__any(pq[qt])) continue;
 #if MCE_PANEL_STATS
                 st_events += 1;
                 const long long t_e0 = clock64();
 #endif
-                const unsigned rem = event(acc[qt], l1[qt], qt, gq[qt], mm[qt] <= rg[qt], jb0, 0xffffu, qlimit_gate);
+                const unsigned rem = event(acc[qt], l1[qt], q0 + qt, gq[q0 + qt], mm[qt] <= rg[q0 + qt], jb0, 0xffffu, qlimit_gate);
                 if (rem) {
-                    if (lane == 0) wredo[nredo] = (int)(rem | ((unsigned)qt << 16) | ((unsigned)tix << 17));
+                    if (lane == 0) wredo[nredo] = (int)(rem | ((unsigned)(q0 + qt) << 16) | ((unsigned)tix << 18));
                     nredo += 1;
                 }
 #if MCE_PANEL_STATS
@@ -524,7 +602,7 @@
 #if MCE_PANEL_STATS
     st_tPro = clock64() - t_kernel0;
 #endif
-    v16f accA[QT], accB[QT];
+    v16f accA[2], accB[2];
     for (int k = 0; k < ntot; ++k) {
         const int buf = k & 1;
         const int c = cfirst + k;
@@ -548,12 +626,12 @@
         const int thi = t_hi - c * CT < CT ? t_hi - c * CT : CT;
         const char* const lbuf = stage0 + buf * CHUNK_BYTES + lane * 16;
         const int jchunk = c * (CT * 32);
-        {
+        if constexpr (QT == 2) {
             v8h a0[KST], a1[KST];
             load_a(lbuf + (tlo * KST) * 1024, a0);
             load_a(lbuf + ((tlo + 1) * KST) * 1024, a1);
-            mfma_first(a0, accA);
-            mfma_rest(a0, accA);
+            mfma_first(a0, accA, 0);
+            mfma_rest(a0, accA, 0);
             int t = tlo;
             float gqP[QT], rgP[QT];
             _Pragma("unroll 1") for (;;)
@@ -566,23 +644,66 @@
                 }
                 const bool more = t + 2 < thi;
                 load_a(lbuf + ((more ? t + 2 : t) * KST) * 1024, a0);
-                mfma_first(a1, accB);
+                mfma_first(a1, accB, 0);
                 MCE_ORDER(accA, accB);
-                mfma_rest(a1, accB);
-                gate_tile(accA, jchunk + t * 32, gqP, rgP, t);
+                mfma_rest(a1, accB, 0);
+                gate_tile(accA, jchunk + t * 32, gqP, rgP, t, 0);
                 if (!more) break;
                 load_a(lbuf + ((t + 3) * KST) * 1024, a1);
-                mfma_first(a0, accA);
+                mfma_first(a0, accA, 0);
                 MCE_ORDER(accB, accA);
-                mfma_rest(a0, accA);
-                gate_tile(accB, jchunk + (t + 1) * 32, gqP, rgP, t + 1);
+                mfma_rest(a0, accA, 0);
+                gate_tile(accB, jchunk + (t + 1) * 32, gqP, rgP, t + 1, 0);
                 t += 2;
             }
             {
 #if defined(__HIP_DEVICE_COMPILE__)
                 asm volatile("s_nop 15\n\ts_nop 3" : "+v"(accB[0]), "+v"(accB[1]));
 #endif
-                gate_tile(accB, jchunk + (t + 1) * 32, gqP, rgP, t + 1);
+                gate_tile(accB, jchunk + (t + 1) * 32, gqP, rgP, t + 1, 0);
+            }
+        } else {
+            v8h a0[KST], a1[KST];
+            load_a(lbuf + (tlo * KST) * 1024, a0);
+            mfma_first(a0, accA, 0);
+            mfma_rest(a0, accA, 0);
+            int t = tlo;
+            float gqP[QT], rgP[QT];
+            _Pragma("unroll 1") for (;;)
+            {
+                const float rP = __uint_as_float((unsigned)__builtin_amdgcn_readlane((int)__float_as_uint(rt_cur), t));
+#pragma unroll
+                for (int qt = 0; qt < QT; ++qt) {
+                    rgP[qt] = rP + cR[qt];
+                    gqP[qt] = vmaxf(G[qt], rgP[qt]);
+                }
+                load_a(lbuf + ((t + 1) * KST) * 1024, a1);
+                mfma_first(a0, accB, 2);
+                MCE_ORDER(accA, accB);
+                mfma_rest(a0, accB, 2);
+                gate_tile(accA, jchunk + t * 32, gqP, rgP, t, 0);
+                mfma_first(a1, accA, 0);
+                MCE_ORDER(accB, accA);
+                mfma_rest(a1, accA, 0);
+                gate_tile(accB, jchunk + t * 32, gqP, rgP, t, 2);
+                const bool more = t + 2 < thi;
+                load_a(lbuf + ((more ? t + 2 : t) * KST) * 1024, a0);
+                mfma_first(a1, accB, 2);
+                MCE_ORDER(accA, accB);
+                mfma_rest(a1, accB, 2);
+                gate_tile(accA, jchunk + (t + 1) * 32, gqP, rgP, t + 1, 0);
+                if (!more) break;
+                mfma_first(a0, accA, 0);
+                MCE_ORDER(accB, accA);
+                mfma_rest(a0, accA, 0);
+                gate_tile(accB, jchunk + (t + 1) * 32, gqP, rgP, t + 1, 2);
+                t += 2;
+            }
+            {
+#if defined(__HIP_DEVICE_COMPILE__)
+                asm volatile("s_nop 15\n\ts_nop 3" : "+v"(accB[0]), "+v"(accB[1]));
+#endif
+                gate_tile(accB, jchunk + (t + 1) * 32, gqP, rgP, t + 1, 2);
             }
         }
         while (need_drain || nredo > 0 || (k + 1 == ntot && qcount > 0)) {
@@ -593,30 +714,40 @@
             for (int i = 0; i < n; ++i) {
                 const unsigned w = (unsigned)__builtin_amdgcn_readfirstlane(wredo[i]);
                 const unsigned todo = w & 0xffffu;
-                const int qt = (int)((w >> 16) & 1u), t = (int)(w >> 17);
+                const int qt = (int)((w >> 16) & 3u), t = (int)(w >> 18);
                 const float Rt = __uint_as_float((unsigned)__builtin_amdgcn_readlane((int)__float_as_uint(rt_cur), t));
                 v8h at[KST];
                 load_a(lbuf + (t * KST) * 1024, at);
                 v16f z = {0.f, 0.f, 0.f, 0.f, 0.f, 0.f, 0.f, 0.f, 0.f, 0.f, 0.f, 0.f, 0.f, 0.f, 0.f, 0.f};
                 v16f r_ = z;
+                float cRq = cR[0], Gq = G[0];
                 if (qt == 0) {
 #pragma unroll
                     for (int ks = 0; ks < KST; ++ks) r_ = __builtin_amdgcn_mfma_f32_32x32x16_f16(at[ks], b[0][ks], r_, 0, 0, 0);
+                } else if (QT == 2 || qt == 1) {
+#pragma unroll
+                    for (int ks = 0; ks < KST; ++ks) r_ = __builtin_amdgcn_mfma_f32_32x32x16_f16(at[ks], b[1][ks], r_, 0, 0, 0);
+                    cRq = cR[1]; Gq = G[1];
+                } else if (qt == 2) {
+#pragma unroll
+                    for (int ks = 0; ks < KST; ++ks) r_ = __builtin_amdgcn_mfma_f32_32x32x16_f16(at[ks], b[QT - 2][ks], r_, 0, 0, 0);
+                    cRq = cR[QT - 2]; Gq = G[QT - 2];
                 } else {
 #pragma unroll
-                    for (int ks = 0; ks < KST; ++ks) r_ = __builtin_amdgcn_mfma_f32_32x32x16_f16(at[ks], b[1][ks], r_, 0, 0, 0);
+                    for (int ks = 0; ks < KST; ++ks) r_ = __builtin_amdgcn_mfma_f32_32x32x16_f16(at[ks], b[QT - 1][ks], r_, 0, 0, 0);
+                    cRq = cR[QT - 1]; Gq = G[QT - 1];
                 }
 #if defined(__HIP_DEVICE_COMPILE__)
                 asm volatile("s_nop 15\n\ts_nop 3" : "+v"(r_));
 #endif
                 float l1[5];
                 const float mm = f16_min16(r_, l1);
-                const float rg = Rt + (qt ? cR[1] : cR[0]);
-                const float gq = vmaxf(qt ? G[1] : G[0], rg);
+                const float rg = Rt + cRq;
+                const float gq = vmaxf(Gq, rg);
                 unsigned rem = 0;
                 if (__any(mm <= gq)) rem = event(r_, l1, qt, gq, mm <= rg, jchunk + t * 32, todo, QN - 64);
                 if (rem) {
-                    if (lane == 0) wredo[nredo] = (int)(rem | ((unsigned)qt << 16) | ((unsigned)t << 17));
+                    if (lane == 0) wredo[nredo] = (int)(rem | ((unsigned)qt << 16) | ((unsigned)t << 18));
                     nredo += 1;
                 }
 #if MCE_PANEL_STATS
@@ -638,17 +769,19 @@
 #endif
     {
         const ArgsPtr a = MCE_ARGS();
-        const int64_t q = qwave0 + lane;
-        const int64_t np = a->nq_pad;
         int chain;
         int64_t list_off;
         chain_of(chain, list_off);
-        const auto pd = gptr_w(a->part_d) + list_off;
-        const auto pi = gptr_w(a->part_i) + list_off;
-#pragma unroll
-        for (int k = 0; k < KCAP; ++k) {
-            pd[(int64_t)k * np + q] = own_d[k];
-            pi[(int64_t)k * np + q] = own_i[k];
+        if constexpr (!LMEM) {
+            const int64_t q = qwave0 + lane;
+            const int64_t np = a->nq_pad;
+            const auto pd = gptr_w(a->part_d) + list_off;
+            const auto pi = gptr_w(a->part_i) + list_off;
+#pragma unroll
+            for (int k = 0; k < KCAP; ++k) {
+                pd[(int64_t)k * np + q] = reg_d[0][k];
+                pi[(int64_t)k * np + q] = reg_i[0][k];
+            }
         }
         __builtin_amdgcn_fence(__ATOMIC_RELEASE, "agent");
         __syncthreads();
```

Result: faster. 28.59 million (median of 6 runs) (+6.6%).
